# NVlabs/latentfusion

Measured on AMD Instinct MI355X. Metric: pose-optim iters/sec (reconstruct+render+backward), 16 views, 128^3 voxels, higher is better.
Workload: dtype f32

## Files before the change

include/lf_hip.h:

```cpp
#ifndef LF_HIP_H
#define LF_HIP_H

#include <stddef.h>
#include <stdint.h>

#ifdef __cplusplus
extern "C" {
#endif

#define LF_ABI_VERSION 1

#define LF_EINVAL   (-1)
#define LF_EALIGN   (-2)
#define LF_ENOSPC   (-3)

#define LF_EPI_LRELU     1u
#define LF_EPI_PIXELNORM 2u
#define LF_EPI_ADD       4u
#define LF_EPI_DOT       8u

#define LF_MAP_O2C 0
#define LF_MAP_C2O 1
#define LF_MAP_COEFS 20

int lf_abi_version(void);

int lf_device_name(char* buf, int buflen);

int lf_resample3d_fwd(const float* vol, int vol_n, const float* coef, int kind,
                      float* out, int N, int D, int H, int W, int C, void* stream);

size_t lf_resample3d_bwd_coef_scratch_bytes(int N, int D, int H, int W);
int lf_resample3d_bwd_coef(const float* gout, const float* vol, int vol_n, const float* coef,
                           float* gcoef, void* scratch, size_t scratch_bytes,
                           int N, int D, int H, int W, int C, void* stream);
size_t lf_resample3d_bwd_coef_part_scratch_bytes(int N, int part_n, int D, int H, int W);
int lf_resample3d_bwd_coef_part(const float* gout, const float* vol, int vol_n, const float* coef,
                                float* gcoef, void* scratch, size_t scratch_bytes,
                                int N, int D, int H, int W, int C, int part_n, void* stream);

int lf_resample3d_fwd_indexed(const float* vol, int vol_n, const int32_t* vol_idx, const float* coef, int kind,
                              float* out, int N, int D, int H, int W, int C, void* stream);
size_t lf_resample3d_bwd_coef_indexed_scratch_bytes(int N, int part_n, int D, int H, int W);
int lf_resample3d_bwd_coef_indexed(const float* gout, const float* vol, int vol_n, const int32_t* vol_idx, const float* coef,
                                   float* gcoef, void* scratch, size_t scratch_bytes,
                                   int N, int D, int H, int W, int C, int part_n, void* stream);


size_t lf_resample3d_bwd_vol_det_scratch_bytes(int vol_n, int D, int H, int W, int C);
int lf_resample3d_bwd_vol_det(const float* gout, const float* coef, int kind, float* gvol, int vol_n, void* scratch,
                              size_t scratch_bytes, int N, int D, int H, int W, int C, void* stream);

int lf_conv3x3_cout_padded(int Cout);
int lf_conv1x1_cout_padded(int Cout);

int lf_conv3x3_fwd(const float* x, const float* wpack, const float* bias, float* y, float* norm_out,
                   int dims, int N, int D, int H, int W, int Cin, int Cout,
                   float he, unsigned flags, float slope, float eps, void* stream);

int lf_conv1x1_fwd(const float* x, const float* wpack, const float* bias, float* y, float* norm_out,
                   int N, int P, int Cin, int ksl, long x_batch_stride, long x_slice_stride,
                   int Cout, long y_batch_stride, int y_row_stride, int y_slice_channels,
                   long y_slice_stride,
                   float he, unsigned flags, float slope, float eps, void* stream);
int lf_conv1x1_fwd_scaled(const float* x, const float* xscale, const float* wpack, const float* bias, float* y, float* norm_out,
                          int N, int P, int Cin, int ksl, long x_batch_stride, long x_slice_stride,
                          int Cout, long y_batch_stride, int y_row_stride, int y_slice_channels,
                          long y_slice_stride,
                          float he, unsigned flags, float slope, float eps, void* stream);

int lf_conv3x3_bwd_data(const float* gy, const float* wpack_t, float* gx, int dims, int N, int D, int H, int W,
                        int Cin, int Cout, float he, const float* prev_y, const float* prev_norm,
                        unsigned prev_flags, float slope, void* stream);
int lf_conv1x1_bwd_data(const float* gy, const float* wpack_t, float* gx, int N, int P, int Cin, int Cout,
                        long y_batch_stride, int y_row_stride, int y_slice_channels, long y_slice_stride,
                        float he, const float* prev_y, const float* prev_norm, unsigned prev_flags,
                        float slope, float* amax_out, void* stream);

#define LF_AMAX_FLOATS 2048
size_t lf_conv3d_c16_split_wpack_halfs(void);
void lf_conv3d_c16_split_pairs(int* taps28);
int lf_conv3d_c16_split(const float* x, const void* wsplit, const float* bias, float* y, float* norm_out,
                        int N, int D, int H, int W, float he, unsigned flags, float slope, float eps,
                        const float* prev_y, const float* prev_norm, unsigned prev_flags,
                        const float* amax_in, float* amax_out, void* stream);

size_t lf_conv3d_c16_wino_upack_floats(void);
int lf_conv3d_c16_wino(const float* x, const float* upack, const float* bias, float* y, float* norm_out,
                       int N, int D, int H, int W, float he, unsigned flags, float slope, float eps,
                       const float* prev_y, const float* prev_norm, unsigned prev_flags,
                       float* amax_out, void* stream);

size_t lf_conv3d_c16_wino_proj_pack_floats(int D);
int lf_conv3d_c16_wino_projfwd(const float* x, const float* upack, const float* bias, float* y, float* norm_out,
                               int N, int D, int H, int W, float he, unsigned flags, float slope, float eps,
                               const float* proj_wA, const float* proj_bias, float* zp, float* pnorm,
                               float proj_he, unsigned proj_flags, void* stream);

int lf_round_bf16(const float* x, float* y, long n, void* stream);
size_t lf_conv3d_c16_ring_bf16_wpack_elems(void);
int lf_conv3d_c16_ring_bf16(const float* x, const void* wpack, const float* bias, float* y, float* norm_out,
                            int N, int D, int H, int W, float he, unsigned flags, float slope, float eps,
                            const float* addend, int round_out, void* stream);
#define LF_IO_IN_BF16 1
#define LF_IO_OUT_BF16 2
#define LF_IO_ADDEND_BF16 4
int lf_conv3d_c16_ring_bf16_io(const void* x, const void* wpack, const float* bias, void* y, float* norm_out,
                               int N, int D, int H, int W, float he, unsigned flags, float slope, float eps,
                               const void* addend, int round_out, int io, void* stream);

#define LF_RING_ADD_BF16 1u
#define LF_RING_OUT_BF16 2u
#define LF_RING_ROUND 4u
#define LF_RING_EX_NONE 0
#define LF_RING_EX_RH 1
#define LF_RING_EX_BLEND 2
#define LF_RING_EX_ABWD 3
#define LF_RING_EX_BLOCK 4
#define LF_RING_EX_PREV 5
int lf_conv3d_c16_ring_multi(const void* x, int x_bf16, const void* wpack, int ngroups,
                             void* y0, const void* add0, unsigned flags0, void* y1, const void* add1, unsigned flags1,
                             int extra, const void* e0, const void* e1, void* o2,
                             int N, int D, int H, int W, float he, int addend_per_sample, void* stream);
int lf_conv3d_c16_ring_blend(const void* rh, const void* wpack, void* cand, const void* addend, const float* h, const void* upre,
                             float* h_new, void* h_new_bf16, int N, int D, int H, int W, float he, void* stream);

long lf_wino3d_tiles(int N, int D, int H, int W);
int lf_wino3d_input_transform(const float* x, float* V, int N, int D, int H, int W, int C, void* stream);

#define LF_OUT_DEPTH_INNER 0x100u
int lf_wino_fused_cout_padded(int Cout);
size_t lf_wino_fused_scratch_bytes(int dims, int N, int D, int H, int W, int Cout);
int lf_wino_fused_gemm(const float* V, const float* U2, const float* bias, float* y, void* scratch, size_t scratch_bytes,
                       int dims, int N, int D, int H, int W, int Cin, int Cout, float he, unsigned flags, float slope,
                       void* stream);

int lf_wino_f16x3_cin_padded(int Cin);
int lf_wino3d_input_transform_f16x3(const float* x, const float* amax_in, void* V, int N, int D, int H, int W, int C, void* stream);
size_t lf_wino_fused_f16x3_scratch_bytes(int N, int D, int H, int W, int Cout);
int lf_wino_fused_f16x3_gemm(const void* V, const void* U2, int eU, const float* amax_in, const float* bias, float* y,
                             float* amax_out, void* scratch, size_t scratch_bytes, int N, int D, int H, int W, int Cin, int Cout,
                             float he, unsigned flags, float slope, void* stream);

long lf_wino2d_tiles(int N, int H, int W);
int lf_wino2d_input_transform(const float* x, float* V, int N, int H, int W, int C, void* stream);

int lf_wino2d_input_transform_f16x3(const float* x, void* V, int* eV, int N, int H, int W, int C, void* stream);
size_t lf_wino_fused2d_f16x3_scratch_bytes(int N, int H, int W, int Cout);
int lf_wino_fused2d_f16x3_gemm(const void* V, const int* eV, const void* U2, int eU, const float* bias, float* y, void* scratch,
                               size_t scratch_bytes, int N, int H, int W, int Cin, int Cout, float he, unsigned flags, float slope,
                               void* stream);

int lf_gru_stage_a(const float* upre, const float* rpre, int pre_stride, const float* h, float* u, float* rec,
                   long nvox, int Ch, int rec_stride, int rec_off, void* stream);
int lf_gru_stage_b(const float* h, const float* u, const float* cand, float* h_out, float* rec, long nvox, int Ch,
                   int rec_stride, int rec_off, void* stream);
int lf_gru_stage_b_bwd(const float* g, const float* h, const float* u, const float* cand, float* gh, float* gu, float* gc,
                       long n, void* stream);
int lf_gru_stage_a_bwd(const float* gu, const float* grh, const float* u, const float* rpre, const float* h, float* gupre,
                       float* grpre, float* gh, long n, void* stream);
int lf_gru_train_stage_a(const void* rpre, const float* h, void* rh, long n, int bf16, void* stream);
int lf_gru_train_stage_b(const float* h, const void* upre, const void* cand, float* h_out, long n, int bf16, void* stream);
int lf_gru_train_stage_b_bwd(const float* g, const float* h, const void* upre, const void* cand, float* gh1, void* gupre,
                             void* gc, float* acc_u, float* acc_o, long n, int bf16, void* stream);
int lf_gru_train_stage_a_bwd(const void* grh, const void* rpre, const float* h, const float* gh1, void* grpre, float* gh12,
                             float* acc_r, long n, int bf16, void* stream);
int lf_sum_views_bf16(const void* src, float* dst, long n, int views, int accumulate, void* stream);

int lf_resample3d_fwd_io(const void* vol, int vol_n, const float* coef, int kind, void* out, int N, int D, int H, int W,
                         int io, void* stream);
size_t lf_resample3d_bwd_vol_det_io_scratch_bytes(int vol_n, int N, int D, int H, int W);
int lf_resample3d_bwd_vol_det_io(const void* gout, const float* coef, int kind, void* gvol, int vol_n, void* scratch,
                                 size_t scratch_bytes, int N, int D, int H, int W, int io, void* stream);

int lf_occ_input_fwd(const float* z, const float* w, const float* b, float* ta, float* t16, int N, int D, long P, float slope,
                     void* stream);
int lf_occ_input_bwd(const float* gta, const float* ta, const float* gp16, const float* w, const float* g_zs, const float* wocc,
                     float* gz, long rows, float slope, const float* prev_y, const float* prev_norm, unsigned prev_flags,
                     void* stream);
int lf_occ_input_bwd_proj(const float* gta, const float* gp16, const float* w, const float* gp2d, const float* wpack_t, float he_p,
                          const float* wocc, float* gz, int N, int D, long P, float slope,
                          const float* prev_y, const float* prev_norm, unsigned prev_flags, void* stream);
int lf_occ_weight_grad(const float* z, const float* gp2d, const float* wpack_t, float he_p, float* gw, int N, int D, long P, void* stream);
int lf_occ_weight_grad_softmax_bwd(const float* z, const float* gp2d, const float* wpack_t, float he_p, const float* weights,
                                   float* glogits, int N, int D, long P, void* stream);
int lf_occ_head_bwd(const float* gl, const float* w16, float he, const float* y, const float* norm, unsigned flags, float slope,
                    float* g, long rows, void* stream);
int lf_occ_conv17_fwd(const float* t16, const float* w27, float* pre, int N, int D, int H, int W, void* stream);
int lf_occ_conv17_bwd(const float* g, const float* t16, const float* w27, float* gp16, int N, int D, int H, int W, float slope,
                      void* stream);
int lf_column_reduce_sum_fwd(const float* x, float* y, int N, int D, long P, int C, void* stream);
int lf_column_reduce_sum_bwd(const float* gy, float* gx, int N, int D, long P, int C, void* stream);
int lf_column_softmax_fwd(const float* logits, float* weights, float* zdepth, int N, int D, long P, void* stream);
int lf_column_softmax_head_fwd(const float* y, const float* w16, const float* bias, float he, float* weights, float* zdepth,
                               int N, int D, long P, void* stream);
int lf_column_softmax_bwd(const float* weights, const float* gweights, const float* gzdepth, float* glogits,
                          int N, int D, long P, void* stream);
int lf_column_scale_fwd(const float* z, const float* w, float* out, long rows, int C, void* stream);
int lf_column_scale_bwd(const float* gout, const float* z, const float* w, float* gz, float* gw, long rows, int C,
                        void* stream);

#define LF_FUSE_MEAN   0
#define LF_FUSE_MAX    1
#define LF_FUSE_ABSMAX 2
#define LF_FUSE_MEDIAN 3
int lf_fuse_views_fwd(const float* z, float* out, int* idx, int kind, int V, long n, long view_stride, void* stream);
int lf_fuse_views_bwd(const float* g, const int* idx, float* gz, int kind, int V, long n, long view_stride, void* stream);
int lf_fuse_blend_fwd(const float* z, const float* logits, float* weights, float* out, int V, long rows, int C,
                      long z_view_stride, long logit_view_stride, void* stream);
int lf_fuse_blend_bwd(const float* g, const float* z, const float* weights, float* gz, float* glogits, int V, long rows,
                      int C, long z_view_stride, long logit_view_stride, void* stream);

int lf_lstm_cell_fwd(const float* cc, const float* c_cur, float* h_next, float* c_next, long nvox, int Ch, void* stream);
int lf_lstm_cell_bwd(const float* cc, const float* c_cur, const float* gh, const float* gcn, float* gcc, float* gc,
                     long nvox, int Ch, void* stream);

int lf_grid_sample2d_fwd(const float* img, const float* grid, float* out, int N, int C, int H, int W, int Ho, int Wo,
                         int bilinear, int border, void* stream);
int lf_grid_sample2d_bwd(const float* img, const float* grid, const float* gout, float* gimg, float* ggrid,
                         int N, int C, int H, int W, int Ho, int Wo, int bilinear, int border, void* stream);

size_t lf_conv_bwd_weight_scratch_bytes(int dims, int N, int D, int H, int W, int Cin, int Cout);
int lf_conv_bwd_weight(const float* x, const float* gpre, float* gw, void* scratch, size_t scratch_bytes,
                       int dims, int N, int D, int H, int W, int Cin, int Cout, float scale, void* stream);
int lf_conv_bwd_weight_bf16(const float* x, const float* gpre, float* gw, void* scratch, size_t scratch_bytes,
                            int dims, int N, int D, int H, int W, int Cin, int Cout, float scale, void* stream);
int lf_conv_bwd_weight_bf16_io(const void* x, const void* gpre, float* gw, void* scratch, size_t scratch_bytes,
                               int dims, int N, int D, int H, int W, int Cin, int Cout, float scale, int io, void* stream);
size_t lf_conv_bwd_weight_wide_scratch_bytes(int dims, int N, int D, int H, int W, int Cin, int Cout);
int lf_conv_bwd_weight_wide(const float* x, const float* gpre, float* gw, void* scratch, size_t scratch_bytes,
                            int dims, int N, int D, int H, int W, int Cin, int Cout, float scale, void* stream);

size_t lf_epilogue_bwd_c16_scratch_bytes(long rows);
int lf_epilogue_bwd_c16(const void* gy, const void* y, const float* norm, void* gp, float* gbias, void* scratch,
                        size_t scratch_bytes, long rows, unsigned flags, float slope, int io, void* stream);

int lf_lift16_fwd(const float* x, const void* wtab, const float* btab, void* vol, float* norm, long R, long P, int S,
                  float he, float slope, float eps, void* stream);
size_t lf_lift16_bwd_scratch_bytes(int S);
int lf_lift16_bwd(const void* gvol, const void* yvol, const float* norm, const float* x, const void* wtab_t, float* gx, float* gw,
                  float* gb, void* scratch, size_t scratch_bytes, long R, long P, int S, float he, float slope, int round_gx,
                  void* stream);

int lf_proj16_fwd(const void* vol, const void* wtab, const float* bias, float* y, float* norm, long R, long P, int S, float he,
                  float slope, float eps, void* stream);
size_t lf_proj16_bwd_scratch_bytes(int S);
int lf_proj16_bwd(const float* gp, const void* vol, const void* wtab_t, void* gxvol, float* gw, void* scratch, size_t scratch_bytes,
                  long R, long P, int S, float he, void* stream);

int lf_pw16_fwd(const void* x, int x_bf16, const void* w_bf16, const float* bias, float he, unsigned flags, float slope, void* y,
                long rows, void* stream);
size_t lf_pw16_bwd_scratch_bytes(long rows);
int lf_pw16_bwd(const void* gy_bf16, const void* wt_bf16, float he, void* gx, int gx_bf16, float* gbias, void* scratch,
                size_t scratch_bytes, long rows, void* stream);

int lf_pixelnorm_fwd(const float* x, float* y, float* norm_out, long rows, int C, float eps, void* stream);

int lf_epilogue_bwd(const float* gy, const float* y, const float* norm, float* gp,
                    long rows, int C, unsigned flags, float slope, void* stream);
int lf_epilogue_bwd_amax(const float* gy, const float* y, const float* norm, float* gp,
                         long rows, int C, unsigned flags, float slope, float* amax_out, void* stream);

int lf_resize_fwd(const float* x, float* y, int dims, int N, int D, int H, int W, int C, int linear, int up,
                  void* stream);
int lf_resize_bwd(const float* gy, float* gx, int dims, int N, int D, int H, int W, int C, int linear, int up,
                  void* stream);

#define LF_CAM_PARAMS 10
#define LF_CAM_COEFS  24
int lf_camera_coefs(const float* params, const float* intrinsics, float cube_size, float z_span,
                    int crop_h, int crop_w, float* coefs, float* jac, int N, void* stream);
int lf_camera_coefs_bwd(const float* gcoefs, const float* jac, float* gparams, int N, void* stream);

size_t lf_pose_loss_scratch_bytes(int N, int h, int w, int H, int W);
int lf_pose_loss_fwd(const float* logits, const float* coefs, const float* target_depth,
                     const float* target_mask, const float* weights, float* sums, float* losses,
                     float* gsums, void* scratch, size_t scratch_bytes,
                     int N, int h, int w, int H, int W, void* stream);
int lf_pose_loss_bwd(const float* logits, const float* coefs, const float* target_depth,
                     const float* target_mask, const float* gsums, float* glogits, float* gcoefs,
                     void* scratch, size_t scratch_bytes, int N, int h, int w, int H, int W, void* stream);
int lf_pose_loss_fwd_masked(const float* logits, const float* coefs, const float* target_depth,
                            const float* target_mask, const float* weights, float* sums, float* losses,
                            void* scratch, size_t scratch_bytes, int N, int h, int w, int H, int W, void* stream);
int lf_pose_loss_fwd_depth(const float* depth_and_logits, const float* coefs, const float* target_depth,
                           const float* target_mask, const float* weights, float* sums, float* losses,
                           float* gsums, void* scratch, size_t scratch_bytes,
                           int N, int h, int w, int H, int W, void* stream);
int lf_pose_loss_bwd_depth(const float* depth_and_logits, const float* coefs, const float* target_depth,
                           const float* target_mask, const float* gsums, float* gcrop, float* gcoefs,
                           void* scratch, size_t scratch_bytes, int N, int h, int w, int H, int W, void* stream);
int lf_pose_loss_fwd_mt(const float* logits, const float* coefs, const float* target_depth,
                        const float* target_mask, const float* weights, float* sums, float* losses,
                        float* gsums, void* scratch, size_t scratch_bytes,
                        int N, int T, int n, int h, int w, int H, int W, void* stream);
int lf_pose_loss_fwd_masked_mt(const float* logits, const float* coefs, const float* target_depth,
                               const float* target_mask, const float* weights, float* sums, float* losses,
                               void* scratch, size_t scratch_bytes, int N, int T, int n, int h, int w, int H, int W,
                               void* stream);
int lf_pose_loss_bwd_mt(const float* logits, const float* coefs, const float* target_depth,
                        const float* target_mask, const float* gsums, float* glogits, float* gcoefs,
                        void* scratch, size_t scratch_bytes, int N, int T, int n, int h, int w, int H, int W,
                        void* stream);

int lf_adam_step(float* params, const float* grads, float* exp_avg, float* exp_avg_sq,
                 const float* step_size, const float* lr, float bias_correction2_sqrt,
                 float beta1, float beta2, float eps, float weight_decay, int N, int P, void* stream);

int lf_nchw_to_nhwc(const float* src, float* dst, int N, int C, long P, void* stream);
int lf_nhwc_to_nchw(const float* src, float* dst, int N, int C, long P, void* stream);
int lf_lift_unfold(const float* src, const float* norm_or_null, float* dst,
                   int N, long P, int C0, int S, void* stream);
int lf_lift_permute(const float* src, float* dst, int N, long P, int C0, int S, int fold, void* stream);
int lf_lift_norm_unfold(const float* src, void* dst, float* norm_out, int N, long P, int C0, int S, float eps, int out_bf16,
                        void* stream);
int lf_lift_bwd(const void* gvol, const void* yvol, const float* norm, float* gp, int N, long P, int C0, int S, float slope,
                int round_bf16, int io, void* stream);

#ifdef __cplusplus
}
#endif
#endif
```

latentfusion_amd/_lib.py:

```python
import ctypes
import os
from ctypes import c_char_p, c_float, c_int, c_long, c_size_t, c_uint, c_void_p

_HERE = os.path.dirname(os.path.abspath(__file__))
LIB_PATH = os.path.join(_HERE, 'csrc', 'liblf_hip.so')

LF_EPI_LRELU = 1
LF_EPI_PIXELNORM = 2
LF_EPI_ADD = 4
LF_EPI_DOT = 8
LF_RING_ADD_BF16, LF_RING_OUT_BF16, LF_RING_ROUND = 1, 2, 4
LF_RING_EX_NONE, LF_RING_EX_RH, LF_RING_EX_BLEND, LF_RING_EX_ABWD, LF_RING_EX_BLOCK, LF_RING_EX_PREV = 0, 1, 2, 3, 4, 5
LF_OUT_DEPTH_INNER = 0x100
LF_IO_IN_BF16, LF_IO_OUT_BF16, LF_IO_ADDEND_BF16 = 1, 2, 4
LF_MAP_O2C = 0
LF_MAP_C2O = 1
LF_MAP_COEFS = 20
LF_FUSE_MEAN, LF_FUSE_MAX, LF_FUSE_ABSMAX, LF_FUSE_MEDIAN = 0, 1, 2, 3
LF_AMAX_FLOATS = 2048

P = c_void_p
SIGNATURES = {
    'lf_abi_version': (c_int, []),
    'lf_device_name': (c_int, [c_char_p, c_int]),
    'lf_resample3d_fwd': (c_int, [P, c_int, P, c_int, P, c_int, c_int, c_int, c_int, c_int, P]),
    'lf_resample3d_bwd_coef_scratch_bytes': (c_size_t, [c_int, c_int, c_int, c_int]),
    'lf_resample3d_bwd_coef': (c_int, [P, P, c_int, P, P, P, c_size_t, c_int, c_int, c_int, c_int, c_int, P]),
    'lf_resample3d_bwd_coef_part_scratch_bytes': (c_size_t, [c_int, c_int, c_int, c_int, c_int]),
    'lf_resample3d_bwd_coef_part': (c_int, [P, P, c_int, P, P, P, c_size_t, c_int, c_int, c_int, c_int, c_int, c_int, P]),
    'lf_resample3d_fwd_indexed': (c_int, [P, c_int, P, P, c_int, P, c_int, c_int, c_int, c_int, c_int, P]),
    'lf_resample3d_bwd_coef_indexed_scratch_bytes': (c_size_t, [c_int, c_int, c_int, c_int, c_int]),
    'lf_resample3d_bwd_coef_indexed': (c_int, [P, P, c_int, P, P, P, P, c_size_t, c_int, c_int, c_int, c_int, c_int, c_int, P]),
    'lf_resample3d_bwd_vol_det_scratch_bytes': (c_size_t, [c_int, c_int, c_int, c_int, c_int]),
    'lf_resample3d_bwd_vol_det': (c_int, [P, P, c_int, P, c_int, P, c_size_t, c_int, c_int, c_int, c_int, c_int, P]),
    'lf_conv3x3_cout_padded': (c_int, [c_int]),
    'lf_conv1x1_cout_padded': (c_int, [c_int]),
    'lf_conv3x3_fwd': (c_int, [P, P, P, P, P, c_int, c_int, c_int, c_int, c_int, c_int, c_int,
                               c_float, c_uint, c_float, c_float, P]),
    'lf_conv1x1_fwd': (c_int, [P, P, P, P, P, c_int, c_int, c_int, c_int, c_long, c_long, c_int, c_long, c_int,
                               c_int, c_long, c_float, c_uint, c_float, c_float, P]),
    'lf_conv1x1_fwd_scaled': (c_int, [P, P, P, P, P, P, c_int, c_int, c_int, c_int, c_long, c_long, c_int, c_long, c_int,
                                      c_int, c_long, c_float, c_uint, c_float, c_float, P]),
    'lf_conv3x3_bwd_data': (c_int, [P, P, P, c_int, c_int, c_int, c_int, c_int, c_int, c_int, c_float, P, P, c_uint,
                                    c_float, P]),
    'lf_conv1x1_bwd_data': (c_int, [P, P, P, c_int, c_int, c_int, c_int, c_long, c_int, c_int, c_long, c_float, P, P,
                                    c_uint, c_float, P, P]),
    'lf_conv3d_c16_split_wpack_halfs': (c_size_t, []),
    'lf_conv3d_c16_split_pairs': (None, [P]),
    'lf_conv3d_c16_split': (c_int, [P, P, P, P, P, c_int, c_int, c_int, c_int, c_float, c_uint, c_float, c_float, P, P,
                                    c_uint, P, P, P]),
    'lf_conv3d_c16_wino_upack_floats': (c_size_t, []),
    'lf_conv3d_c16_wino': (c_int, [P, P, P, P, P, c_int, c_int, c_int, c_int, c_float, c_uint, c_float, c_float, P, P,
                                   c_uint, P, P]),
    'lf_conv3d_c16_wino_proj_pack_floats': (c_size_t, [c_int]),
    'lf_conv3d_c16_wino_projfwd': (c_int, [P, P, P, P, P, c_int, c_int, c_int, c_int, c_float, c_uint, c_float, c_float,
                                           P, P, P, P, c_float, c_uint, P]),
    'lf_round_bf16': (c_int, [P, P, c_long, P]),
    'lf_conv3d_c16_ring_bf16_wpack_elems': (c_size_t, []),
    'lf_conv3d_c16_ring_bf16': (c_int, [P, P, P, P, P, c_int, c_int, c_int, c_int, c_float, c_uint, c_float, c_float, P, c_int, P]),
    'lf_conv3d_c16_ring_bf16_io': (c_int, [P, P, P, P, P, c_int, c_int, c_int, c_int, c_float, c_uint, c_float, c_float, P, c_int, c_int, P]),
    'lf_conv3d_c16_ring_multi': (c_int, [P, c_int, P, c_int, P, P, c_uint, P, P, c_uint, c_int, P, P, P, c_int, c_int, c_int, c_int, c_float, c_int, P]),
    'lf_conv3d_c16_ring_blend': (c_int, [P, P, P, P, P, P, P, P, c_int, c_int, c_int, c_int, c_float, P]),
    'lf_wino3d_tiles': (c_long, [c_int, c_int, c_int, c_int]),
    'lf_wino3d_input_transform': (c_int, [P, P, c_int, c_int, c_int, c_int, c_int, P]),
    'lf_wino_fused_cout_padded': (c_int, [c_int]),
    'lf_wino_fused_scratch_bytes': (c_size_t, [c_int, c_int, c_int, c_int, c_int, c_int]),
    'lf_wino_fused_gemm': (c_int, [P, P, P, P, P, c_size_t, c_int, c_int, c_int, c_int, c_int, c_int, c_int, c_float, c_uint, c_float, P]),
    'lf_wino_f16x3_cin_padded': (c_int, [c_int]),
    'lf_wino3d_input_transform_f16x3': (c_int, [P, P, P, c_int, c_int, c_int, c_int, c_int, P]),
    'lf_wino_fused_f16x3_scratch_bytes': (c_size_t, [c_int, c_int, c_int, c_int, c_int]),
    'lf_wino_fused_f16x3_gemm': (c_int, [P, P, c_int, P, P, P, P, P, c_size_t, c_int, c_int, c_int, c_int, c_int, c_int,
                                         c_float, c_uint, c_float, P]),
    'lf_wino2d_tiles': (c_long, [c_int, c_int, c_int]),
    'lf_wino2d_input_transform': (c_int, [P, P, c_int, c_int, c_int, c_int, P]),
    'lf_wino2d_input_transform_f16x3': (c_int, [P, P, P, c_int, c_int, c_int, c_int, P]),
    'lf_wino_fused2d_f16x3_scratch_bytes': (c_size_t, [c_int, c_int, c_int, c_int]),
    'lf_wino_fused2d_f16x3_gemm': (c_int, [P, P, P, c_int, P, P, P, c_size_t, c_int, c_int, c_int, c_int, c_int, c_float, c_uint,
                                           c_float, P]),
    'lf_gru_stage_a': (c_int, [P, P, c_int, P, P, P, c_long, c_int, c_int, c_int, P]),
    'lf_gru_stage_b': (c_int, [P, P, P, P, P, c_long, c_int, c_int, c_int, P]),
    'lf_lstm_cell_fwd': (c_int, [P, P, P, P, c_long, c_int, P]),
    'lf_lstm_cell_bwd': (c_int, [P, P, P, P, P, P, c_long, c_int, P]),
    'lf_gru_stage_b_bwd': (c_int, [P, P, P, P, P, P, P, c_long, P]),
    'lf_gru_stage_a_bwd': (c_int, [P, P, P, P, P, P, P, P, c_long, P]),
    'lf_gru_train_stage_a': (c_int, [P, P, P, c_long, c_int, P]),
    'lf_gru_train_stage_b': (c_int, [P, P, P, P, c_long, c_int, P]),
    'lf_gru_train_stage_b_bwd': (c_int, [P, P, P, P, P, P, P, P, P, c_long, c_int, P]),
    'lf_gru_train_stage_a_bwd': (c_int, [P, P, P, P, P, P, P, c_long, c_int, P]),
    'lf_lift16_fwd': (c_int, [P, P, P, P, P, c_long, c_long, c_int, c_float, c_float, c_float, P]),
    'lf_lift16_bwd_scratch_bytes': (c_size_t, [c_int]),
    'lf_lift16_bwd': (c_int, [P, P, P, P, P, P, P, P, P, c_size_t, c_long, c_long, c_int, c_float, c_float, c_int, P]),
    'lf_proj16_fwd': (c_int, [P, P, P, P, P, c_long, c_long, c_int, c_float, c_float, c_float, P]),
    'lf_proj16_bwd_scratch_bytes': (c_size_t, [c_int]),
    'lf_proj16_bwd': (c_int, [P, P, P, P, P, P, c_size_t, c_long, c_long, c_int, c_float, P]),
    'lf_sum_views_bf16': (c_int, [P, P, c_long, c_int, c_int, P]),
    'lf_occ_input_fwd': (c_int, [P, P, P, P, P, c_int, c_int, c_long, c_float, P]),
    'lf_occ_input_bwd': (c_int, [P, P, P, P, P, P, P, c_long, c_float, P, P, c_uint, P]),
    'lf_occ_conv17_fwd': (c_int, [P, P, P, c_int, c_int, c_int, c_int, P]),
    'lf_occ_conv17_bwd': (c_int, [P, P, P, P, c_int, c_int, c_int, c_int, c_float, P]),
    'lf_column_reduce_sum_fwd': (c_int, [P, P, c_int, c_int, c_long, c_int, P]),
    'lf_column_reduce_sum_bwd': (c_int, [P, P, c_int, c_int, c_long, c_int, P]),
    'lf_column_softmax_fwd': (c_int, [P, P, P, c_int, c_int, c_long, P]),
    'lf_occ_input_bwd_proj': (c_int, [P, P, P, P, P, c_float, P, P, c_int, c_int, c_long, c_float, P, P, c_uint, P]),
    'lf_occ_weight_grad': (c_int, [P, P, P, c_float, P, c_int, c_int, c_long, P]),
    'lf_pw16_fwd': (c_int, [P, c_int, P, P, c_float, c_uint, c_float, P, c_long, P]),
    'lf_pw16_bwd_scratch_bytes': (c_size_t, [c_long]),
    'lf_pw16_bwd': (c_int, [P, P, c_float, P, c_int, P, P, c_size_t, c_long, P]),
    'lf_occ_weight_grad_softmax_bwd': (c_int, [P, P, P, c_float, P, P, c_int, c_int, c_long, P]),
    'lf_occ_head_bwd': (c_int, [P, P, c_float, P, P, c_uint, c_float, P, c_long, P]),
    'lf_column_softmax_head_fwd': (c_int, [P, P, P, c_float, P, P, c_int, c_int, c_long, P]),
    'lf_column_softmax_bwd': (c_int, [P, P, P, P, c_int, c_int, c_long, P]),
    'lf_column_scale_fwd': (c_int, [P, P, P, c_long, c_int, P]),
    'lf_column_scale_bwd': (c_int, [P, P, P, P, P, c_long, c_int, P]),
    'lf_fuse_views_fwd': (c_int, [P, P, P, c_int, c_int, c_long, c_long, P]),
    'lf_fuse_views_bwd': (c_int, [P, P, P, c_int, c_int, c_long, c_long, P]),
    'lf_fuse_blend_fwd': (c_int, [P, P, P, P, c_int, c_long, c_int, c_long, c_long, P]),
    'lf_fuse_blend_bwd': (c_int, [P, P, P, P, P, c_int, c_long, c_int, c_long, c_long, P]),
    'lf_grid_sample2d_fwd': (c_int, [P, P, P, c_int, c_int, c_int, c_int, c_int, c_int, c_int, c_int, P]),
    'lf_grid_sample2d_bwd': (c_int, [P, P, P, P, P, c_int, c_int, c_int, c_int, c_int, c_int, c_int, c_int, P]),
    'lf_conv_bwd_weight_scratch_bytes': (c_size_t, [c_int, c_int, c_int, c_int, c_int, c_int, c_int]),
    'lf_conv_bwd_weight': (c_int, [P, P, P, P, c_size_t, c_int, c_int, c_int, c_int, c_int, c_int, c_int, c_float, P]),
    'lf_conv_bwd_weight_bf16': (c_int, [P, P, P, P, c_size_t, c_int, c_int, c_int, c_int, c_int, c_int, c_int, c_float, P]),
    'lf_conv_bwd_weight_bf16_io': (c_int, [P, P, P, P, c_size_t, c_int, c_int, c_int, c_int, c_int, c_int, c_int, c_float, c_int, P]),
    'lf_conv_bwd_weight_wide_scratch_bytes': (c_size_t, [c_int, c_int, c_int, c_int, c_int, c_int, c_int]),
    'lf_conv_bwd_weight_wide': (c_int, [P, P, P, P, c_size_t, c_int, c_int, c_int, c_int, c_int, c_int, c_int, c_float, P]),
    'lf_pixelnorm_fwd': (c_int, [P, P, P, c_long, c_int, c_float, P]),
    'lf_epilogue_bwd': (c_int, [P, P, P, P, c_long, c_int, c_uint, c_float, P]),
    'lf_epilogue_bwd_amax': (c_int, [P, P, P, P, c_long, c_int, c_uint, c_float, P, P]),
    'lf_epilogue_bwd_c16_scratch_bytes': (c_size_t, [c_long]),
    'lf_epilogue_bwd_c16': (c_int, [P, P, P, P, P, P, c_size_t, c_long, c_uint, c_float, c_int, P]),
    'lf_resample3d_fwd_io': (c_int, [P, c_int, P, c_int, P, c_int, c_int, c_int, c_int, c_int, P]),
    'lf_resample3d_bwd_vol_det_io_scratch_bytes': (c_size_t, [c_int, c_int, c_int, c_int, c_int]),
    'lf_resample3d_bwd_vol_det_io': (c_int, [P, P, c_int, P, c_int, P, c_size_t, c_int, c_int, c_int, c_int, c_int, P]),
    'lf_resize_fwd': (c_int, [P, P, c_int, c_int, c_int, c_int, c_int, c_int, c_int, c_int, P]),
    'lf_resize_bwd': (c_int, [P, P, c_int, c_int, c_int, c_int, c_int, c_int, c_int, c_int, P]),
    'lf_camera_coefs': (c_int, [P, P, c_float, c_float, c_int, c_int, P, P, c_int, P]),
    'lf_camera_coefs_bwd': (c_int, [P, P, P, c_int, P]),
    'lf_pose_loss_scratch_bytes': (c_size_t, [c_int, c_int, c_int, c_int, c_int]),
    'lf_pose_loss_fwd': (c_int, [P, P, P, P, P, P, P, P, P, c_size_t, c_int, c_int, c_int, c_int, c_int, P]),
    'lf_pose_loss_bwd': (c_int, [P, P, P, P, P, P, P, P, c_size_t, c_int, c_int, c_int, c_int, c_int, P]),
    'lf_pose_loss_fwd_depth': (c_int, [P, P, P, P, P, P, P, P, P, c_size_t, c_int, c_int, c_int, c_int, c_int, P]),
    'lf_pose_loss_bwd_depth': (c_int, [P, P, P, P, P, P, P, P, c_size_t, c_int, c_int, c_int, c_int, c_int, P]),
    'lf_pose_loss_fwd_masked': (c_int, [P, P, P, P, P, P, P, P, c_size_t, c_int, c_int, c_int, c_int, c_int, P]),
    'lf_pose_loss_fwd_mt': (c_int, [P, P, P, P, P, P, P, P, P, c_size_t, c_int, c_int, c_int, c_int, c_int, c_int, c_int, P]),
    'lf_pose_loss_fwd_masked_mt': (c_int, [P, P, P, P, P, P, P, P, c_size_t, c_int, c_int, c_int, c_int, c_int, c_int, c_int,
                                           P]),
    'lf_pose_loss_bwd_mt': (c_int, [P, P, P, P, P, P, P, P, c_size_t, c_int, c_int, c_int, c_int, c_int, c_int, c_int, P]),
    'lf_adam_step': (c_int, [P, P, P, P, P, P, c_float, c_float, c_float, c_float, c_float, c_int, c_int, P]),
    'lf_nchw_to_nhwc': (c_int, [P, P, c_int, c_int, c_long, P]),
    'lf_nhwc_to_nchw': (c_int, [P, P, c_int, c_int, c_long, P]),
    'lf_lift_unfold': (c_int, [P, P, P, c_int, c_long, c_int, c_int, P]),
    'lf_lift_permute': (c_int, [P, P, c_int, c_long, c_int, c_int, c_int, P]),
    'lf_lift_norm_unfold': (c_int, [P, P, P, c_int, c_long, c_int, c_int, c_float, c_int, P]),
    'lf_lift_bwd': (c_int, [P, P, P, P, c_int, c_long, c_int, c_int, c_float, c_int, c_int, P]),
}

EXPERIMENTAL_SIGNATURES = {
    'lf_set_tuning': (c_int, [c_int, c_int]),
    'lf_resample3d_bwd_vol': (c_int, [P, P, c_int, P, c_int, c_int, c_int, c_int, c_int, c_int, P]),
    'lf_conv3d_c16_wino_projbwd': (c_int, [P, P, c_float, P, P, c_uint, P, P, c_int, c_int, c_int, c_int, c_float, c_float,
                                           P, P, c_uint, P]),
    'lf_conv3d_c16_wino_split_upack_halfs': (c_size_t, []),
    'lf_conv3d_c16_wino_split': (c_int, [P, P, P, P, P, c_int, c_int, c_int, c_int, c_float, c_uint, c_float, c_float, P, P,
                                         c_uint, P, P, P]),
    'lf_conv3d_c16_bf16_wpack_elems': (c_size_t, []),
    'lf_conv3d_c16_bf16': (c_int, [P, P, P, P, P, c_int, c_int, c_int, c_int, c_float, c_uint, c_float, c_float, c_int, P]),
    'lf_wino3d_output_transform': (c_int, [P, P, P, P, c_int, c_int, c_int, c_int, c_int, c_float, c_uint, c_float, c_float, P]),
    'lf_wino2d_output_transform': (c_int, [P, P, P, P, c_int, c_int, c_int, c_int, c_float, c_uint, c_float, c_float, P]),
}

_lib = None


class LFHipError(RuntimeError):
    pass


def lib():
    global _lib
    if _lib is not None:
        return _lib
    if not os.path.exists(LIB_PATH):
        try:
            from .csrc import build as _build
            _build.build(verbose=False)
        except Exception as e:
            raise LFHipError(f'liblf_hip.so is missing at {LIB_PATH} and could not be built: {e}') from e
    import torch
    try:
        handle = ctypes.CDLL(LIB_PATH)
    except OSError as e:
        raise LFHipError(f'cannot load {LIB_PATH}: {e}') from e
    for name, (res, args) in list(SIGNATURES.items()) + list(EXPERIMENTAL_SIGNATURES.items()):
        try:
            fn = getattr(handle, name)
        except AttributeError as e:
            raise LFHipError(f'{LIB_PATH} does not export {name}') from e
        fn.restype = res
        fn.argtypes = args
    if handle.lf_abi_version() != 1:
        raise LFHipError('liblf_hip.so ABI version mismatch')
    _lib = handle
    return _lib


_ERR = {-1: 'LF_EINVAL (bad size/flag combination)', -2: 'LF_EALIGN (alignment / channel count)',
        -3: 'LF_ENOSPC (scratch too small)'}


BYTE_LOG = None
_PENDING = [0]


def note_bytes(t, scratch=False):
    if BYTE_LOG is not None and not scratch:
        n = t.numel() * t.element_size()
        try:
            n = min(n, t.untyped_storage().nbytes() - t.storage_offset() * t.element_size())
        except Exception:
            pass
        _PENDING[0] += n


def check(rc, what):
    if BYTE_LOG is not None:
        e = BYTE_LOG.setdefault(what, [0, 0])
        e[0] += 1
        e[1] += _PENDING[0]
        _PENDING[0] = 0
    if rc != 0:
        raise LFHipError(f'{what} failed: {_ERR.get(rc, "hipError " + str(rc))}')
```

latentfusion_amd/csrc/build.py:

```python
import os
import subprocess
import sys

HERE = os.path.dirname(os.path.abspath(__file__))
SOURCES = ['resample.hip', 'conv.hip', 'pointwise.hip', 'image.hip', 'optim.hip', 'resize.hip', 'conv_split.hip', 'conv_wino.hip', 'wgrad.hip', 'sample2d.hip', 'gru.hip', 'wino_gemm.hip', 'reduce.hip', 'wino_fused.hip', 'conv_bf16.hip', 'occlusion.hip', 'conv_gru.hip', 'lift_mfma.hip', 'pw16.hip', 'wino_fused_f16x3.hip', 'wgrad_wide.hip']
LIB = os.path.join(HERE, 'liblf_hip.so')
EXTRA = {'conv_split.hip': ['-fno-slp-vectorize'], 'conv_gru.hip': ['-fno-slp-vectorize']}
FLAGS = ['--offload-arch=gfx950', '-O3', '-std=c++17', '-fPIC', '-fno-gpu-rdc', '-Wall', '-Wno-unused-function']


def _hipcc():
    for cand in (os.environ.get('HIPCC'), '/opt/rocm/bin/hipcc', 'hipcc'):
        if cand and (os.path.isabs(cand) and os.path.exists(cand) or not os.path.isabs(cand)):
            return cand
    raise RuntimeError('hipcc not found')


def needs_build():
    if not os.path.exists(LIB):
        return True
    t = os.path.getmtime(LIB)
    deps = [os.path.join(HERE, s) for s in SOURCES if os.path.exists(os.path.join(HERE, s))]
    deps += [os.path.join(HERE, f) for f in os.listdir(HERE) if f.endswith(('.h', '.inc'))]
    deps += [os.path.join(HERE, '..', '..', 'include', 'lf_hip.h'), os.path.join(HERE, '..', '..', 'include', 'lf_hip_experimental.h')]
    return any(os.path.getmtime(d) > t for d in deps)


def build(force=False, verbose=True):
    if not force and not needs_build():
        return LIB
    hipcc = _hipcc()
    objs = []
    procs = []
    for src in SOURCES:
        path = os.path.join(HERE, src)
        if not os.path.exists(path):
            continue
        obj = os.path.join(HERE, src.replace('.hip', '.o'))
        objs.append(obj)
        cmd = [hipcc, '-x', 'hip', '-c', path, '-o', obj] + FLAGS + EXTRA.get(src, [])
        procs.append((cmd, subprocess.Popen(cmd, stdout=subprocess.PIPE, stderr=subprocess.STDOUT)))
    for cmd, p in procs:
        out, _ = p.communicate()
        if p.returncode != 0:
            raise RuntimeError('hipcc failed: ' + ' '.join(cmd) + '\n' + out.decode())
        if verbose and out.strip():
            print(out.decode())
    cmd = [hipcc, '-shared', '-fPIC', '--offload-arch=gfx950', '-o', LIB] + objs
    r = subprocess.run(cmd, stdout=subprocess.PIPE, stderr=subprocess.STDOUT)
    if r.returncode != 0:
        raise RuntimeError('link failed:\n' + r.stdout.decode())
    if verbose:
        print('built', LIB)
    return LIB


if __name__ == '__main__':
    build(force='--force' in sys.argv)
```

latentfusion_amd/csrc/lf_common.h:

```cpp
#pragma once
#include <hip/hip_runtime.h>
#include <stdint.h>
#include "../../include/lf_hip.h"
#include "../../include/lf_hip_experimental.h"

#define LF_WAVE 64

typedef float f32x4 __attribute__((ext_vector_type(4)));

static inline void lf_clear_error() { (void)hipGetLastError(); }

static inline int lf_launch_status() {
  hipError_t e = hipGetLastError();
  return (int)e;
}

static inline bool lf_aligned16(const void* p) { return (((uintptr_t)p) & 15u) == 0; }

#include <atomic>
typedef std::atomic<unsigned long long> lf_devmask_t;
static inline hipError_t lf_ensure_dyn_lds(lf_devmask_t& done, const void* fn, int bytes) {
  int dev = 0;
  if (hipGetDevice(&dev) != hipSuccess) dev = 0;
  const unsigned long long bit = 1ull << (dev & 63);
  if (done.load(std::memory_order_acquire) & bit) return hipSuccess;
  const hipError_t e = hipFuncSetAttribute(fn, hipFuncAttributeMaxDynamicSharedMemorySize, bytes);
  if (e == hipSuccess) done.fetch_or(bit, std::memory_order_release);
  return e;
}

__device__ __forceinline__ float lf_wave_sum(float v) {
#pragma unroll
  for (int o = 32; o > 0; o >>= 1) v += __shfl_xor(v, o, 64);
  return v;
}

#define LF_AMAX_SLOTS 64
#define LF_AMAX_STRIDE 32
static_assert(LF_AMAX_FLOATS == LF_AMAX_SLOTS * LF_AMAX_STRIDE, "lf_hip.h: LF_AMAX_FLOATS");

__device__ __forceinline__ void lf_amax_publish(float* base, float wave_max, int lane) {
  if (lane == 0 && wave_max > 0.f)
    atomicMax((unsigned int*)(base + (blockIdx.x % LF_AMAX_SLOTS) * LF_AMAX_STRIDE), __float_as_uint(wave_max));
}

__device__ __forceinline__ float lf_amax_read(const float* base, int lane) {
  float m = base[(lane % LF_AMAX_SLOTS) * LF_AMAX_STRIDE];
#pragma unroll
  for (int o = 32; o > 0; o >>= 1) m = fmaxf(m, __shfl_xor(m, o, 64));
  return m;
}

__device__ __forceinline__ float lf_lrelu(float v, float slope) { return v > 0.f ? v : v * slope; }

int lf_internal_ring_bf16_set_wgs(int v);
int lf_internal_fused_set_cfg(int v);
```

latentfusion_amd/csrc/resample.hip:

```cpp
#include "lf_common.h"
#include <type_traits>

namespace {

typedef unsigned u32x4_t __attribute__((ext_vector_type(4)));

struct Tap {
  int x0, y0, z0, x1, y1, z1;
  float tx, ty, tz;
  float mx, my, mz;
};

__device__ __forceinline__ float lattice01(int i, int size, float step) {
  return (i < size / 2) ? step * (float)i : 1.f - step * (float)(size - 1 - i);
}

struct Steps { float w, h, d; };

template <int KIND>
__device__ __forceinline__ void eval_grid(const float* __restrict__ cf, int x, int y, int z,
                                          int W, int H, int D, Steps st, float& gx, float& gy, float& gz,
                                          float& a, float& b, float& k) {
  a = lattice01(x, W, st.w);
  b = lattice01(y, H, st.h);
  k = lattice01(z, D, st.d);
  if (KIND == LF_MAP_O2C) {
    const float ak = a * k, bk = b * k;
    gx = cf[0] + cf[3] * a + cf[6] * b + cf[9] * k + cf[12] * ak + cf[15] * bk;
    gy = cf[1] + cf[4] * a + cf[7] * b + cf[10] * k + cf[13] * ak + cf[16] * bk;
    gz = cf[2] + cf[5] * a + cf[8] * b + cf[11] * k + cf[14] * ak + cf[17] * bk;
  } else {
    const float lx = 2.f * a - 1.f, ly = 2.f * b - 1.f, lz = 2.f * k - 1.f;
    const float n0 = cf[0] * lx + cf[1] * ly + cf[2] * lz + cf[3];
    const float n1 = cf[4] * lx + cf[5] * ly + cf[6] * lz + cf[7];
    const float n2 = cf[8] * lx + cf[9] * ly + cf[10] * lz + cf[11];
    const float dn = cf[12] * lx + cf[13] * ly + cf[14] * lz + cf[15];
    gx = n0 / dn;
    gy = n1 / dn;
    gz = n2;
  }
}

__device__ __forceinline__ void unnormalize_clip(float g, int size, float& pos, float& mult) {
  float p = ((g + 1.f) * (float)size - 1.f) * 0.5f;
  const float hi = (float)(size - 1);
  mult = (p > 0.f && p < hi) ? 0.5f * (float)size : 0.f;
  p = fminf(fmaxf(p, 0.f), hi);
  pos = p;
}

__device__ __forceinline__ Tap make_tap(float gx, float gy, float gz, int W, int H, int D) {
  Tap t;
  float px, py, pz;
  unnormalize_clip(gx, W, px, t.mx);
  unnormalize_clip(gy, H, py, t.my);
  unnormalize_clip(gz, D, pz, t.mz);
  if (!(px == px)) px = 0.f;
  if (!(py == py)) py = 0.f;
  if (!(pz == pz)) pz = 0.f;
  const float fx = floorf(px), fy = floorf(py), fz = floorf(pz);
  t.tx = px - fx; t.ty = py - fy; t.tz = pz - fz;
  t.x0 = (int)fx; t.y0 = (int)fy; t.z0 = (int)fz;
  t.x1 = min(t.x0 + 1, W - 1); t.y1 = min(t.y0 + 1, H - 1); t.z1 = min(t.z0 + 1, D - 1);
  return t;
}

__device__ __forceinline__ unsigned xcd_contiguous(unsigned b, unsigned nb) {
  return (nb % 8 == 0) ? (b % 8) * (nb / 8) + b / 8 : b;
}

static int bwd_vox_per_block(long nvox, int N) {
  long v = nvox * N / 2048;
  int p = 64;
  while (p < 4096 && p * 2 <= v) p <<= 1;
  return p;
}
struct BwdTile { int lx, ly, lz, ntx, nty, ntz; };
static BwdTile bwd_tile(int vpb, int D, int H, int W) {
  int lg = 0;
  while ((1 << lg) < vpb) ++lg;
  BwdTile t;
  t.lx = (lg + 2) / 3; t.ly = (lg + 1) / 3; t.lz = lg / 3;
  t.ntx = (W + (1 << t.lx) - 1) >> t.lx; t.nty = (H + (1 << t.ly) - 1) >> t.ly; t.ntz = (D + (1 << t.lz) - 1) >> t.lz;
  return t;
}

__global__ void __launch_bounds__(256) resample_bwd_coef_reduce(const float* __restrict__ partial,
                                                                int nblk, float* __restrict__ gcoef) {
  const int n = blockIdx.x;
  __shared__ double red[256];
  const int comp = threadIdx.x % 18;
  const int grp = threadIdx.x / 18;
  double s = 0.0;
  if (grp < 14)
    for (int b = grp; b < nblk; b += 14) s += (double)partial[((long)n * nblk + b) * 18 + comp];
  red[threadIdx.x] = (grp < 14) ? s : 0.0;
  __syncthreads();
  if (threadIdx.x < 18) {
    double tot = 0.0;
    for (int g = 0; g < 14; ++g) tot += red[g * 18 + threadIdx.x];
    gcoef[(long)n * 18 + threadIdx.x] = (float)tot;
  }
}

template <int KIND>
__global__ void __launch_bounds__(256) resample_bwd_vol_kernel(
    const float* __restrict__ gout, const float* __restrict__ coef, float* __restrict__ gvol,
    long gvol_bstride, int N, int D, int H, int W, int C, Steps st) {
  const long per_sample = (long)D * H * W * C;
  const int n = blockIdx.y;
  const float* cf = coef + (long)n * LF_MAP_COEFS;
  for (long idx = (long)blockIdx.x * blockDim.x + threadIdx.x; idx < per_sample;
       idx += (long)gridDim.x * blockDim.x) {
    const int c = (int)(idx % C);
    long v = idx / C;
    const int x = (int)(v % W); v /= W;
    const int y = (int)(v % H);
    const int z = (int)(v / H);
    float gx, gy, gz, a, b, k;
    eval_grid<KIND>(cf, x, y, z, W, H, D, st, gx, gy, gz, a, b, k);
    const Tap t = make_tap(gx, gy, gz, W, H, D);
    const float go = gout[(long)n * per_sample + idx];
    float* base = gvol + (long)n * gvol_bstride + c;
    const long sW = C, sH = (long)W * C, sD = (long)H * W * C;
    const float wx1 = t.tx, wx0 = 1.f - t.tx, wy1 = t.ty, wy0 = 1.f - t.ty, wz1 = t.tz, wz0 = 1.f - t.tz;
    atomicAdd(base + t.z0 * sD + t.y0 * sH + t.x0 * sW, go * (wx0 * wy0 * wz0));
    atomicAdd(base + t.z0 * sD + t.y0 * sH + t.x1 * sW, go * (wx1 * wy0 * wz0));
    atomicAdd(base + t.z0 * sD + t.y1 * sH + t.x0 * sW, go * (wx0 * wy1 * wz0));
    atomicAdd(base + t.z0 * sD + t.y1 * sH + t.x1 * sW, go * (wx1 * wy1 * wz0));
    atomicAdd(base + t.z1 * sD + t.y0 * sH + t.x0 * sW, go * (wx0 * wy0 * wz1));
    atomicAdd(base + t.z1 * sD + t.y0 * sH + t.x1 * sW, go * (wx1 * wy0 * wz1));
    atomicAdd(base + t.z1 * sD + t.y1 * sH + t.x0 * sW, go * (wx0 * wy1 * wz1));
    atomicAdd(base + t.z1 * sD + t.y1 * sH + t.x1 * sW, go * (wx1 * wy1 * wz1));
  }
}

typedef unsigned u32;

struct Tap32 {
  u32 o000, o001, o010, o011, o100, o101, o110, o111;
  float tx, ty, tz, mx, my, mz;
};

__device__ __forceinline__ void axis_tap(float g, int size, u32 stride, u32& o0, u32& d1, float& t, float& m) {
  float p;
  unnormalize_clip(g, size, p, m);
  if (!(p == p)) p = 0.f;
  const float f = floorf(p);
  t = p - f;
  const int i0 = (int)f;
  o0 = (u32)i0 * stride;
  d1 = (i0 + 1 <= size - 1) ? stride : 0u;
}

__device__ __forceinline__ Tap32 make_tap32(float gx, float gy, float gz, int W, int H, int D, u32 rec_bytes) {
  Tap32 t;
  u32 x0, dx, y0, dy, z0, dz;
  axis_tap(gx, W, rec_bytes, x0, dx, t.tx, t.mx);
  axis_tap(gy, H, rec_bytes * (u32)W, y0, dy, t.ty, t.my);
  axis_tap(gz, D, rec_bytes * (u32)W * (u32)H, z0, dz, t.tz, t.mz);
  const u32 b00 = z0 + y0, b01 = b00 + dy, b10 = b00 + dz, b11 = b01 + dz;
  t.o000 = b00 + x0; t.o001 = t.o000 + dx;
  t.o010 = b01 + x0; t.o011 = t.o010 + dx;
  t.o100 = b10 + x0; t.o101 = t.o100 + dx;
  t.o110 = b11 + x0; t.o111 = t.o110 + dx;
  return t;
}

__device__ __forceinline__ f32x4 ldrec(__amdgpu_buffer_rsrc_t rs, u32 off) {
  return __builtin_bit_cast(f32x4, __builtin_amdgcn_raw_buffer_load_b128(rs, (int)off, 0, 0));
}

typedef __bf16 bf16x4r __attribute__((ext_vector_type(4)));
typedef unsigned u32x2_t __attribute__((ext_vector_type(2)));
template <bool B16>
__device__ __forceinline__ f32x4 ldrec_t(__amdgpu_buffer_rsrc_t rs, u32 off) {
  if constexpr (B16)
    return __builtin_convertvector(__builtin_bit_cast(bf16x4r, __builtin_amdgcn_raw_buffer_load_b64(rs, (int)off, 0, 0)), f32x4);
  else
    return __builtin_bit_cast(f32x4, __builtin_amdgcn_raw_buffer_load_b128(rs, (int)off, 0, 0));
}

__device__ __forceinline__ float quad_sum4(float v) {
  const float a = v + __int_as_float(__builtin_amdgcn_update_dpp(0, __float_as_int(v), 0xB1, 0xF, 0xF, true));
  return a + __int_as_float(__builtin_amdgcn_update_dpp(0, __float_as_int(a), 0x4E, 0xF, 0xF, true));
}

__device__ __forceinline__ long vol_offset(int n, long vol_bstride, const int* __restrict__ vol_idx, int vol_n) {
  const int v = vol_idx[n];
  return (long)(v < 0 ? 0 : (v >= vol_n ? vol_n - 1 : v)) * vol_bstride;
}

#define GATHER_KERNEL(stem) stem##_kernel
#define GATHER_TABLE_PARAMS
#define GATHER_VOL_OFFSET ((long)n * vol_bstride)
#include "resample_gather.inc"
#undef GATHER_KERNEL
#undef GATHER_TABLE_PARAMS
#undef GATHER_VOL_OFFSET
#define GATHER_KERNEL(stem) stem##_indexed_kernel
#define GATHER_TABLE_PARAMS const int* __restrict__ vol_idx, int vol_n,
#define GATHER_VOL_OFFSET vol_offset(n, vol_bstride, vol_idx, vol_n)
#include "resample_gather.inc"
#undef GATHER_KERNEL
#undef GATHER_TABLE_PARAMS
#undef GATHER_VOL_OFFSET

template <int KIND>
__global__ void __launch_bounds__(256) resample_fwd_c16_dedup_kernel(
    const float* __restrict__ vol, long vol_bstride, const float* __restrict__ coef,
    float* __restrict__ out, int D, int H, int W, int nbx, int nby, int nbz, Steps st) {
  __shared__ u32x4_t tapo[4][64];
  __shared__ f32x4 tapf[4][64];
  const int lane = threadIdx.x & 63, wave = threadIdx.x >> 6;
  const int n = blockIdx.z / nbz, bz = blockIdx.z - n * nbz;
  const int x0 = ((blockIdx.x << 2) + wave) << 2, y0 = blockIdx.y << 2, z0 = bz << 2;
  const u32 sample_bytes = (u32)D * (u32)H * (u32)W * 64u;
  const __amdgpu_buffer_rsrc_t rs = __builtin_amdgcn_make_buffer_rsrc((void*)(vol + (long)n * vol_bstride), 0, sample_bytes, 0x00020000);
  const __amdgpu_buffer_rsrc_t ro = __builtin_amdgcn_make_buffer_rsrc((void*)(out + (long)n * D * H * W * 16), 0, sample_bytes, 0x00020000);
  const float* cf = coef + n * LF_MAP_COEFS;
  {
    const int x = x0 + (lane & 3), y = y0 + ((lane >> 2) & 3), z = z0 + (lane >> 4);
    const bool live = x < W && y < H && z < D;
    float gx, gy, gz, a, b, k;
    eval_grid<KIND>(cf, live ? x : 0, live ? y : 0, live ? z : 0, W, H, D, st, gx, gy, gz, a, b, k);
    const Tap32 t = make_tap32(gx, gy, gz, W, H, D, 64u);
    u32x4_t o;
    o[0] = live ? t.o000 : 0xffffffffu;
    o[1] = t.o001 - t.o000; o[2] = t.o010 - t.o000; o[3] = t.o100 - t.o000;
    tapo[wave][lane] = o;
    tapf[wave][lane] = (f32x4){t.tx, t.ty, t.tz, 0.f};
  }
  asm volatile("s_waitcnt lgkmcnt(0)" ::: "memory");
  const int q = lane & 3, vq = lane >> 2;
  const u32 co = (u32)q * 16u;
#pragma unroll
  for (int i = 0; i < 4; ++i) {
    const int vi = 16 * i + vq;
    const u32x4_t o = tapo[wave][vi];
    const f32x4 f = tapf[wave][vi];
    if (o[0] == 0xffffffffu) continue;
    const u32 b00 = o[0] + co, b01 = b00 + o[2], b10 = b00 + o[3], b11 = b01 + o[3];
    const f32x4 v000 = ldrec(rs, b00), v001 = ldrec(rs, b00 + o[1]), v010 = ldrec(rs, b01), v011 = ldrec(rs, b01 + o[1]);
    const f32x4 v100 = ldrec(rs, b10), v101 = ldrec(rs, b10 + o[1]), v110 = ldrec(rs, b11), v111 = ldrec(rs, b11 + o[1]);
    const float wx1 = f[0], wx0 = 1.f - f[0], wy1 = f[1], wy0 = 1.f - f[1], wz1 = f[2], wz0 = 1.f - f[2];
    const float w000 = wx0 * wy0 * wz0, w001 = wx1 * wy0 * wz0, w010 = wx0 * wy1 * wz0, w011 = wx1 * wy1 * wz0;
    const float w100 = wx0 * wy0 * wz1, w101 = wx1 * wy0 * wz1, w110 = wx0 * wy1 * wz1, w111 = wx1 * wy1 * wz1;
    f32x4 r;
#pragma unroll
    for (int e = 0; e < 4; ++e) {
      float acc = v000[e] * w000;
      asm("v_fmac_f32 %0, %1, %2" : "+v"(acc) : "v"(v001[e]), "v"(w001));
      asm("v_fmac_f32 %0, %1, %2" : "+v"(acc) : "v"(v010[e]), "v"(w010));
      asm("v_fmac_f32 %0, %1, %2" : "+v"(acc) : "v"(v011[e]), "v"(w011));
      asm("v_fmac_f32 %0, %1, %2" : "+v"(acc) : "v"(v100[e]), "v"(w100));
// ... 562 lines not shown
  for (int j = 0; j < 16; ++j) {
    const int r = wv * 64 + j * 4 + grp;
    const int lx = r % STX, ly = (r / STX) % STY, lz = r / (STX * STY);
    const int x = tx0 + lx, y = ty0 + ly, z = tz0 + lz;
    if (x < W && y < H && z < D) {
      char* dst = (char*)gvol + (n_out * nvox + (((long)z * H + y) * W + x)) * OREC;
      const float o = (float)((double)(long long)acc[r * 16 + ch] * inv);
      if constexpr (OUT16) ((__bf16*)dst)[ch] = __builtin_convertvector((f32x4){o, o, o, o}, bf16x4r)[0];
      else ((float*)dst)[ch] = o;
    }
  }
}

int g_splat_chunk_cap = 0;
inline int splat_bin_chunk(int N, long nvox) {
  long cv = (512L << 20) / (nvox * 32);
  if (cv < 1) cv = 1;
  if (g_splat_chunk_cap > 0 && cv > g_splat_chunk_cap) cv = g_splat_chunk_cap;
  return (int)(cv < N ? cv : N);
}

int g_splat_variant = 2;

bool pow2(int v) { return v > 0 && (v & (v - 1)) == 0; }

Steps make_steps(int D, int H, int W) {
  Steps st;
  st.w = W > 1 ? 1.0f / (float)(W - 1) : 0.f;
  st.h = H > 1 ? 1.0f / (float)(H - 1) : 0.f;
  st.d = D > 1 ? 1.0f / (float)(D - 1) : 0.f;
  return st;
}

}

struct FwdPlan {
  bool vec;
  int lpt, tlx, tly, tlz, nbz;
  dim3 grid;
  Steps st;
};
static int fwd_plan(const float* vol, const float* out, int N, int D, int H, int W, int C, FwdPlan& p) {
  if ((long)D * H * W >= 0x7fffffffL) return LF_EINVAL;
  p.vec = (C % 4 == 0) && lf_aligned16(vol) && lf_aligned16(out);
  const int lpv = p.vec ? C / 4 : C;
  p.lpt = lpv < 256 ? lpv : 256;
  int lg = 0;
  while ((2 << lg) * p.lpt <= 256) ++lg;
  if (lg >= 6) { p.tlx = (lg + 2) / 3; p.tly = (lg + 1) / 3; p.tlz = lg / 3; }
  else         { p.tlx = lg < 2 ? lg : 2; p.tly = lg - p.tlx < 2 ? lg - p.tlx : 2; p.tlz = lg - p.tlx - p.tly; }
  p.nbz = (D + (1 << p.tlz) - 1) >> p.tlz;
  const int nby = (H + (1 << p.tly) - 1) >> p.tly;
  if ((long)p.nbz * N > 65535 || nby > 65535) return LF_EINVAL;
  p.grid = dim3((unsigned)((W + (1 << p.tlx) - 1) >> p.tlx), (unsigned)nby, (unsigned)(p.nbz * N));
  p.st = make_steps(D, H, W);
  return 0;
}

#define LAUNCH_BY_KIND(KERNEL, GRID, ...)                                                                   \
  do {                                                                                                      \
    if (kind == LF_MAP_O2C) hipLaunchKernelGGL((KERNEL<LF_MAP_O2C>), GRID, dim3(256), 0, s, __VA_ARGS__);   \
    else                    hipLaunchKernelGGL((KERNEL<LF_MAP_C2O>), GRID, dim3(256), 0, s, __VA_ARGS__);   \
  } while (0)
extern "C" int lf_resample3d_fwd(const float* vol, int vol_n, const float* coef, int kind, float* out,
                                 int N, int D, int H, int W, int C, void* stream) {
  lf_clear_error();
  if (N <= 0 || D <= 0 || H <= 0 || W <= 0 || C <= 0) return LF_EINVAL;
  if (vol_n != 1 && vol_n != N) return LF_EINVAL;
  if (kind != LF_MAP_O2C && kind != LF_MAP_C2O) return LF_EINVAL;
  const long bstride = vol_n == 1 ? 0 : (long)D * H * W * C;
  FwdPlan p;
  if (int e = fwd_plan(vol, out, N, D, H, W, C, p)) return e;
  hipStream_t s = (hipStream_t)stream;
  if (g_resample_variant == 4 && p.vec && C == 16 && (long)D * H * W * 64 < 0xffffffffL && W <= 65535) {
    const int ntx = (W + LT_X - 1) / LT_X, nty = (H + LT_Y - 1) / LT_Y, ntz = (D + LT_Z - 1) / LT_Z;
    const long nwg = (long)ntx * nty * ntz * N;
    if (nwg > 0x7fffffffL) return LF_EINVAL;
    LAUNCH_BY_KIND(resample_fwd_staged_kernel, dim3((unsigned)nwg), vol, bstride, coef, out, D, H, W, ntx, nty, ntz, p.st);
    return lf_launch_status();
  }
  if (g_resample_variant == 5 && p.vec && C == 16 && (long)D * H * W * 64 < 0xffffffffL) {
    const int nbz4 = (D + 3) >> 2, nbx16 = (W + 15) >> 4, nby4 = (H + 3) >> 2;
    if ((long)nbz4 * N > 65535 || nby4 > 65535) return LF_EINVAL;
    dim3 g5((unsigned)nbx16, (unsigned)nby4, (unsigned)(nbz4 * N));
    LAUNCH_BY_KIND(resample_fwd_c16_dedup_kernel, g5, vol, bstride, coef, out, D, H, W, nbx16, nby4, nbz4, p.st);
    return lf_launch_status();
  }
  if (g_resample_variant >= 3 && p.vec && C == 16 && (long)D * H * W * 64 < 0xffffffffL) {
    LAUNCH_BY_KIND(resample_fwd_c16_kernel, p.grid, vol, bstride, coef, out, D, H, W, p.nbz, p.st);
  } else if (g_resample_variant >= 2 && p.vec && (long)D * H * W * C * 4 < 0xffffffffL) {
    LAUNCH_BY_KIND(resample_fwd_lean_kernel, p.grid, vol, bstride, coef, out, D, H, W, C, p.lpt, p.tlx, p.tly, p.tlz, p.nbz, p.st);
  } else {
#define LAUNCH(K, V) hipLaunchKernelGGL((resample_fwd_kernel<K, V>), p.grid, dim3(256), 0, s, vol, bstride, coef, out, N, D, H, W, C, p.lpt, p.tlx, p.tly, p.tlz, p.nbz, p.st)
    if (kind == LF_MAP_O2C) { if (p.vec) LAUNCH(LF_MAP_O2C, 4); else LAUNCH(LF_MAP_O2C, 1); }
    else                    { if (p.vec) LAUNCH(LF_MAP_C2O, 4); else LAUNCH(LF_MAP_C2O, 1); }
#undef LAUNCH
  }
  return lf_launch_status();
}

static long staged_bwd_blocks(int D, int H, int W) {
  const long nt = (long)((W + LT_X - 1) / LT_X) * ((H + LT_Y - 1) / LT_Y) * ((D + LT_Z - 1) / LT_Z);
  return (nt + STAGED_TPW - 1) / STAGED_TPW;
}

static size_t bwd_coef_scratch_bytes(int N, int part_n, int D, int H, int W) {
  const long nvox = (long)D * H * W;
  const int vpb = bwd_vox_per_block(nvox, part_n);
  const BwdTile bt = bwd_tile(vpb, D, H, W);
  const long nblk = (long)bt.ntx * bt.nty * bt.ntz;
  const long nblk_staged = staged_bwd_blocks(D, H, W);
  return (size_t)N * (nblk > nblk_staged ? nblk : nblk_staged) * 18 * sizeof(float);
}

extern "C" size_t lf_resample3d_bwd_coef_scratch_bytes(int N, int D, int H, int W) {
  return bwd_coef_scratch_bytes(N, N, D, H, W);
}

extern "C" size_t lf_resample3d_bwd_coef_part_scratch_bytes(int N, int part_n, int D, int H, int W) {
  if (N <= 0 || part_n <= 0) return 0;
  return bwd_coef_scratch_bytes(N, part_n, D, H, W);
}

struct BwdCoefPlan {
  long nvox;
  int vpb, nblk, lpv;
  BwdTile bt;
  bool vec;
  dim3 grid;
  Steps st;
};
static int bwd_coef_plan(const float* gout, const float* vol, size_t scratch_bytes, int N, int part_n, int D, int H, int W, int C,
                         BwdCoefPlan& p) {
  if (scratch_bytes < bwd_coef_scratch_bytes(N, part_n, D, H, W)) return LF_ENOSPC;
  if ((long)D * H * W >= 0x7fffffffL) return LF_EINVAL;
  p.nvox = (long)D * H * W;
  p.vpb = bwd_vox_per_block(p.nvox, part_n);
  p.bt = bwd_tile(p.vpb, D, H, W);
  const long nblk_l = (long)p.bt.ntx * p.bt.nty * p.bt.ntz;
  if (nblk_l * N > 0x7fffffffL) return LF_EINVAL;
  p.nblk = (int)nblk_l;
  p.grid = dim3((unsigned)(nblk_l * N));
  p.vec = (C % 4 == 0) && lf_aligned16(gout) && lf_aligned16(vol);
  const int groups = p.vec ? C / 4 : C;
  p.lpv = 1;
  while (p.lpv < groups) p.lpv <<= 1;
  if (p.lpv > 64) return LF_EINVAL;
  p.st = make_steps(D, H, W);
  return 0;
}

static int bwd_coef_finish(const float* partial, int nblk, float* gcoef, int N, hipStream_t s) {
  if (int e = lf_launch_status()) return e;
  hipLaunchKernelGGL(resample_bwd_coef_reduce, dim3(N), dim3(256), 0, s, partial, nblk, gcoef);
  return lf_launch_status();
}

static int bwd_coef_launch(const float* gout, const float* vol, int vol_n, const float* coef,
                           float* gcoef, void* scratch, size_t scratch_bytes,
                           int N, int part_n, int D, int H, int W, int C, void* stream) {
  if (N <= 0 || D <= 0 || H <= 0 || W <= 0 || C <= 0) return LF_EINVAL;
  if (vol_n != 1 && vol_n != N) return LF_EINVAL;
  BwdCoefPlan p;
  if (int e = bwd_coef_plan(gout, vol, scratch_bytes, N, part_n, D, H, W, C, p)) return e;
  const long bstride = vol_n == 1 ? 0 : p.nvox * C;
  hipStream_t s = (hipStream_t)stream;
  float* partial = (float*)scratch;
  if (g_resample_variant == 4 && p.vec && C == 16 && p.nvox * 64 < 0xffffffffL && W <= 65535) {
    const int ntx = (W + LT_X - 1) / LT_X, nty = (H + LT_Y - 1) / LT_Y, ntz = (D + LT_Z - 1) / LT_Z;
    const long nb = staged_bwd_blocks(D, H, W);
    if (nb * N > 0x7fffffffL) return LF_EINVAL;
    hipLaunchKernelGGL((resample_bwd_coef_staged_kernel<STAGED_TPW>), dim3((unsigned)(nb * N)), dim3(256), 0, s, gout, vol, bstride, coef,
                       partial, (int)nb, D, H, W, ntx, nty, ntz, p.st);
    return bwd_coef_finish(partial, (int)nb, gcoef, N, s);
  }
  if (g_resample_variant >= 2 && p.vec && C == 16 && p.vpb >= 64 && p.nvox * 64 < 0xffffffffL) {
    const int v = g_bwd_coef_variant;
    const bool big = p.vpb >= 256;
#define LAUNCH(...) hipLaunchKernelGGL((__VA_ARGS__), p.grid, dim3(256), 0, s, gout, vol, bstride, coef, partial, p.nblk, p.vpb, p.bt, D, H, W, p.st)
    if (v == 1)              LAUNCH(resample_bwd_coef_c16_kernel<1, 1>);
    else if (v == 2)         LAUNCH(resample_bwd_coef_c16_kernel<1, 2>);
    else if (v == 3)         LAUNCH(resample_bwd_coef_c16_kernel<4, 2>);
    else if (v == 6 && big)  LAUNCH(resample_bwd_coef_c16_dedup_kernel<2, 1>);
    else if (v == 7 && big)  LAUNCH(resample_bwd_coef_c16_dedup_kernel<1, 1>);
    else if (v == 8 && big)  LAUNCH(resample_bwd_coef_c16_dedup_kernel<2, 4>);
    else if (v == 9 && big)  LAUNCH(resample_bwd_coef_c16_dedup_kernel<1, 5>);
    else if (v == 10 && big) LAUNCH(resample_bwd_coef_c16_dedup_kernel<2, 1, true>);
    else if (v == 11 && big) LAUNCH(resample_bwd_coef_c16_dedup_kernel<1, 1, true>);
    else if (v == 4)         LAUNCH(resample_bwd_coef_c16_kernel<6, 1>);
    else                     LAUNCH(resample_bwd_coef_c16_kernel<8, 1>);
#undef LAUNCH
  } else if (p.vec) {
    hipLaunchKernelGGL((resample_bwd_coef_kernel<4>), p.grid, dim3(256), 0, s, gout, vol, bstride, coef, partial, p.nblk, p.vpb, p.bt, N, D, H, W, C, p.lpv, p.st);
  } else {
    hipLaunchKernelGGL((resample_bwd_coef_kernel<1>), p.grid, dim3(256), 0, s, gout, vol, bstride, coef, partial, p.nblk, p.vpb, p.bt, N, D, H, W, C, p.lpv, p.st);
  }
  return bwd_coef_finish(partial, p.nblk, gcoef, N, s);
}

extern "C" int lf_resample3d_bwd_coef(const float* gout, const float* vol, int vol_n, const float* coef,
                                      float* gcoef, void* scratch, size_t scratch_bytes,
                                      int N, int D, int H, int W, int C, void* stream) {
  lf_clear_error();
  return bwd_coef_launch(gout, vol, vol_n, coef, gcoef, scratch, scratch_bytes, N, N, D, H, W, C, stream);
}

extern "C" int lf_resample3d_bwd_coef_part(const float* gout, const float* vol, int vol_n, const float* coef,
                                           float* gcoef, void* scratch, size_t scratch_bytes,
                                           int N, int D, int H, int W, int C, int part_n, void* stream) {
  lf_clear_error();
  if (!gout || !vol || !coef || !gcoef || !scratch) return LF_EINVAL;
  if (part_n <= 0 || N <= 0) return LF_EINVAL;
  return bwd_coef_launch(gout, vol, vol_n, coef, gcoef, scratch, scratch_bytes, N, part_n, D, H, W, C, stream);
}

extern "C" int lf_resample3d_fwd_indexed(const float* vol, int vol_n, const int* vol_idx, const float* coef, int kind, float* out,
                                         int N, int D, int H, int W, int C, void* stream) {
  lf_clear_error();
  if (!vol || !vol_idx || !coef || !out) return LF_EINVAL;
  if (N <= 0 || D <= 0 || H <= 0 || W <= 0 || C <= 0 || vol_n < 1) return LF_EINVAL;
  if (kind != LF_MAP_O2C && kind != LF_MAP_C2O) return LF_EINVAL;
  if (((uintptr_t)vol_idx & 3) != 0) return LF_EALIGN;
  const long bstride = (long)D * H * W * C;
  FwdPlan p;
  if (int e = fwd_plan(vol, out, N, D, H, W, C, p)) return e;
  hipStream_t s = (hipStream_t)stream;
  if (g_resample_variant >= 3 && p.vec && C == 16 && (long)D * H * W * 64 < 0xffffffffL) {
    LAUNCH_BY_KIND(resample_fwd_c16_indexed_kernel, p.grid, vol, bstride, vol_idx, vol_n, coef, out, D, H, W, p.nbz, p.st);
  } else if (g_resample_variant >= 2 && p.vec && (long)D * H * W * C * 4 < 0xffffffffL) {
    LAUNCH_BY_KIND(resample_fwd_lean_indexed_kernel, p.grid, vol, bstride, vol_idx, vol_n, coef, out, D, H, W, C, p.lpt, p.tlx, p.tly, p.tlz, p.nbz, p.st);
  } else {
#define LAUNCH(K, V) hipLaunchKernelGGL((resample_fwd_indexed_kernel<K, V>), p.grid, dim3(256), 0, s, vol, bstride, vol_idx, vol_n, coef, out, N, D, H, W, C, p.lpt, p.tlx, p.tly, p.tlz, p.nbz, p.st)
    if (kind == LF_MAP_O2C) { if (p.vec) LAUNCH(LF_MAP_O2C, 4); else LAUNCH(LF_MAP_O2C, 1); }
    else                    { if (p.vec) LAUNCH(LF_MAP_C2O, 4); else LAUNCH(LF_MAP_C2O, 1); }
#undef LAUNCH
  }
  return lf_launch_status();
}
#undef LAUNCH_BY_KIND

extern "C" size_t lf_resample3d_bwd_coef_indexed_scratch_bytes(int N, int part_n, int D, int H, int W) {
  if (N <= 0 || part_n <= 0) return 0;
  return bwd_coef_scratch_bytes(N, part_n, D, H, W);
}

extern "C" int lf_resample3d_bwd_coef_indexed(const float* gout, const float* vol, int vol_n, const int* vol_idx, const float* coef,
                                              float* gcoef, void* scratch, size_t scratch_bytes,
                                              int N, int D, int H, int W, int C, int part_n, void* stream) {
  lf_clear_error();
  if (!gout || !vol || !vol_idx || !coef || !gcoef || !scratch) return LF_EINVAL;
  if (part_n <= 0 || N <= 0 || vol_n < 1) return LF_EINVAL;
  if (D <= 0 || H <= 0 || W <= 0 || C <= 0) return LF_EINVAL;
  if (((uintptr_t)vol_idx & 3) != 0) return LF_EALIGN;
  BwdCoefPlan p;
  if (int e = bwd_coef_plan(gout, vol, scratch_bytes, N, part_n, D, H, W, C, p)) return e;
  const long bstride = p.nvox * C;
  hipStream_t s = (hipStream_t)stream;
  float* partial = (float*)scratch;
  if (g_resample_variant >= 2 && p.vec && C == 16 && p.vpb >= 64 && p.nvox * 64 < 0xffffffffL) {
    if (p.vpb >= 256)
      hipLaunchKernelGGL((resample_bwd_coef_c16_dedup_indexed_kernel<2, 1, true>), p.grid, dim3(256), 0, s, gout, vol, bstride, vol_idx, vol_n, coef, partial, p.nblk, p.vpb, p.bt, D, H, W, p.st);
    else
      hipLaunchKernelGGL((resample_bwd_coef_c16_indexed_kernel<8, 1>), p.grid, dim3(256), 0, s, gout, vol, bstride, vol_idx, vol_n, coef, partial, p.nblk, p.vpb, p.bt, D, H, W, p.st);
  } else if (p.vec) {
    hipLaunchKernelGGL((resample_bwd_coef_indexed_kernel<4>), p.grid, dim3(256), 0, s, gout, vol, bstride, vol_idx, vol_n, coef, partial, p.nblk, p.vpb, p.bt, N, D, H, W, C, p.lpv, p.st);
  } else {
    hipLaunchKernelGGL((resample_bwd_coef_indexed_kernel<1>), p.grid, dim3(256), 0, s, gout, vol, bstride, vol_idx, vol_n, coef, partial, p.nblk, p.vpb, p.bt, N, D, H, W, C, p.lpv, p.st);
  }
  return bwd_coef_finish(partial, p.nblk, gcoef, N, s);
}

extern "C" int lf_resample3d_bwd_vol(const float* gout, const float* coef, int kind, float* gvol, int vol_n,
                                     int N, int D, int H, int W, int C, void* stream) {
  lf_clear_error();
  if (N <= 0 || D <= 0 || H <= 0 || W <= 0 || C <= 0) return LF_EINVAL;
  if (vol_n != 1 && vol_n != N) return LF_EINVAL;
  const long bstride = vol_n == 1 ? 0 : (long)D * H * W * C;
  const long items = (long)D * H * W * C;
  dim3 grid((unsigned)min((items + 255) / 256, (long)65535 * 16), N), block(256);
  hipStream_t s = (hipStream_t)stream;
  if (kind == LF_MAP_O2C)
    hipLaunchKernelGGL((resample_bwd_vol_kernel<LF_MAP_O2C>), grid, block, 0, s, gout, coef, gvol, bstride, N, D, H, W, C, make_steps(D, H, W));
  else if (kind == LF_MAP_C2O)
    hipLaunchKernelGGL((resample_bwd_vol_kernel<LF_MAP_C2O>), grid, block, 0, s, gout, coef, gvol, bstride, N, D, H, W, C, make_steps(D, H, W));
  else
    return LF_EINVAL;
  return lf_launch_status();
}

#ifdef STAGE_TS
extern "C" int lf_debug_stage_ts(void* dst) {
  return (int)hipMemcpyFromSymbol(dst, HIP_SYMBOL(g_stage_ts), sizeof(unsigned long long) * 256 * 16, 0, hipMemcpyDeviceToHost);
}
#endif

extern "C" int lf_set_tuning(int key, int value) {
  if (key == 1) {
    const int prev = g_resample_variant;
    if (value >= 1 && value <= 5) g_resample_variant = value;
    return prev;
  }
  if (key == 4) {
    const int prev = g_splat_variant;
    if (value >= 1 && value <= 4) g_splat_variant = value;
    return prev;
  }
  if (key == 6) {
    const int prev = g_splat_chunk_cap;
    if (value >= 0) g_splat_chunk_cap = value;
    return prev;
  }
  if (key == 3) return lf_internal_fused_set_cfg(value);
  if (key == 5) return lf_internal_ring_bf16_set_wgs(value);
  if (key == 2) {
    const int prev = g_bwd_coef_variant;
    if (value >= 1 && value <= 11) g_bwd_coef_variant = value;
    return prev;
  }
  return LF_EINVAL;
}

extern "C" size_t lf_resample3d_bwd_vol_det_scratch_bytes(int vol_n, int D, int H, int W, int C) {
  if (vol_n <= 0 || D <= 0 || H <= 0 || W <= 0 || C <= 0) return 0;
  return (size_t)vol_n * D * H * W * C * sizeof(long long) + 256;
}

extern "C" int lf_resample3d_bwd_vol_det(const float* gout, const float* coef, int kind, float* gvol, int vol_n, void* scratch,
                                         size_t scratch_bytes, int N, int D, int H, int W, int C, void* stream) {
  lf_clear_error();
  if (N <= 0 || D <= 0 || H <= 0 || W <= 0 || C <= 0) return LF_EINVAL;
  if ((vol_n != 1 && vol_n != N) || (kind != LF_MAP_O2C && kind != LF_MAP_C2O)) return LF_EINVAL;
  const long items = (long)D * H * W * C, total = items * vol_n;
  if (scratch == nullptr || scratch_bytes < lf_resample3d_bwd_vol_det_scratch_bytes(vol_n, D, H, W, C)) return LF_ENOSPC;
  if ((((uintptr_t)scratch) & 7u) != 0) return LF_EALIGN;
  hipStream_t s = (hipStream_t)stream;
  const long ng = items * N;
  const int nbx = (W + 3) / 4, nby = (H + 3) / 4, nbz = (D + 3) / 4;
  const long nblk = (long)nbx * nby * nbz;
  const int ntx = (W + STX - 1) / STX, nty = (H + STY - 1) / STY, ntz = (D + STZ - 1) / STZ;
  const int nsx = (nbx + 3) / 4, nsy = (nby + 3) / 4, nsz = (nbz + 3) / 4, nsb = nsx * nsy * nsz;
  if (g_splat_variant >= 2 && C == 16 && lf_aligned16(gout) && lf_aligned16(gvol) && D < 0x7fff && H < 0x7fff && W < 0x7fff &&
      nblk < 0x7fffffffL / 4 && (long)ntx * nty * ntz < 0x7fffffffL && N <= 65535 &&
      scratch_bytes >= 256 + (size_t)N * (nblk + nsb) * sizeof(uint3)) {
    unsigned* amax = (unsigned*)scratch;
    uint3* bbox = (uint3*)((char*)scratch + 256);
    uint3* sbox = bbox + (size_t)N * nblk;
    hipError_t e = hipMemsetAsync(scratch, 0, 256, s);
    if (e != hipSuccess) return (int)e;
    hipLaunchKernelGGL(absmax_kernel, dim3((unsigned)min((ng + 255) / 256, 4096L)), dim3(256), 0, s, gout, ng, amax);
    const Steps stp = make_steps(D, H, W);
    const dim3 gb((unsigned)((nblk + 3) / 4), (unsigned)N), gs2((unsigned)((nsb + 3) / 4), (unsigned)N),
        gt((unsigned)((long)ntx * nty * ntz), (unsigned)vol_n);
    if (kind == LF_MAP_O2C)
      hipLaunchKernelGGL((splat_bbox_kernel<LF_MAP_O2C>), gb, dim3(256), 0, s, coef, bbox, (int)nblk, nbx, nby, D, H, W, stp);
    else
      hipLaunchKernelGGL((splat_bbox_kernel<LF_MAP_C2O>), gb, dim3(256), 0, s, coef, bbox, (int)nblk, nbx, nby, D, H, W, stp);
    hipLaunchKernelGGL(splat_bbox2_kernel, gs2, dim3(256), 0, s, bbox, sbox, (int)nblk, nsb, nbx, nby, nbz, nsx, nsy);
    if (kind == LF_MAP_O2C)
      hipLaunchKernelGGL((splat_tile_kernel<LF_MAP_O2C>), gt, dim3(256), 0, s, gout, coef, bbox, sbox, amax, gvol, vol_n, N, (int)nblk, nsb,
                         nbx, nby, nbz, nsx, nsy, ntx, nty, D, H, W, stp);
    else
      hipLaunchKernelGGL((splat_tile_kernel<LF_MAP_C2O>), gt, dim3(256), 0, s, gout, coef, bbox, sbox, amax, gvol, vol_n, N, (int)nblk, nsb,
                         nbx, nby, nbz, nsx, nsy, ntx, nty, D, H, W, stp);
    return lf_launch_status();
  }
  unsigned long long* acc = (unsigned long long*)scratch;
  unsigned* amax = (unsigned*)((char*)scratch + (size_t)total * sizeof(long long));
  hipError_t e = hipMemsetAsync(scratch, 0, (size_t)total * sizeof(long long) + 256, s);
  if (e != hipSuccess) return (int)e;
  hipLaunchKernelGGL(absmax_kernel, dim3((unsigned)min((ng + 255) / 256, 4096L)), dim3(256), 0, s, gout, ng, amax);
  int st = lf_launch_status();
  if (st) return st;
  const long bstride = vol_n == 1 ? 0 : items;
  dim3 grid((unsigned)min((items + 255) / 256, (long)65535 * 16), N), block(256);
  if (kind == LF_MAP_O2C)
    hipLaunchKernelGGL((resample_bwd_vol_fixed_kernel<LF_MAP_O2C>), grid, block, 0, s, gout, coef, acc, bstride, amax, N, D, H, W, C, make_steps(D, H, W));
  else
    hipLaunchKernelGGL((resample_bwd_vol_fixed_kernel<LF_MAP_C2O>), grid, block, 0, s, gout, coef, acc, bstride, amax, N, D, H, W, C, make_steps(D, H, W));
  st = lf_launch_status();
  if (st) return st;
  hipLaunchKernelGGL(fixed_to_float_kernel, dim3((unsigned)((total + 255) / 256)), dim3(256), 0, s, (const long long*)acc, amax, gvol, total);
  return lf_launch_status();
}

extern "C" int lf_resample3d_fwd_io(const void* vol, int vol_n, const float* coef, int kind, void* out,
                                    int N, int D, int H, int W, int io, void* stream) {
  lf_clear_error();
  if (N <= 0 || D <= 0 || H <= 0 || W <= 0 || io < 0 || io > 3) return LF_EINVAL;
  if ((vol_n != 1 && vol_n != N) || (kind != LF_MAP_O2C && kind != LF_MAP_C2O)) return LF_EINVAL;
  if (!lf_aligned16(vol) || !lf_aligned16(out)) return LF_EALIGN;
  if ((long)D * H * W * 64 >= 0xffffffffL) return LF_EINVAL;
  const long bstride = vol_n == 1 ? 0 : (long)D * H * W * 16;
  const int nbz4 = (D + 3) >> 2;
  if ((long)nbz4 * N > 65535 || ((H + 3) >> 2) > 65535) return LF_EINVAL;
  dim3 g4((unsigned)((W + 3) >> 2), (unsigned)((H + 3) >> 2), (unsigned)(nbz4 * N)), block(256);
  const Steps st = make_steps(D, H, W);
  typedef void (*kern_t)(const float*, long, const float*, float*, int, int, int, int, Steps);
  static const kern_t kerns[2][4] = {
      {resample_fwd_c16_kernel<LF_MAP_O2C, 0>, resample_fwd_c16_kernel<LF_MAP_O2C, 1>, resample_fwd_c16_kernel<LF_MAP_O2C, 2>, resample_fwd_c16_kernel<LF_MAP_O2C, 3>},
      {resample_fwd_c16_kernel<LF_MAP_C2O, 0>, resample_fwd_c16_kernel<LF_MAP_C2O, 1>, resample_fwd_c16_kernel<LF_MAP_C2O, 2>, resample_fwd_c16_kernel<LF_MAP_C2O, 3>}};
  hipLaunchKernelGGL(kerns[kind == LF_MAP_O2C ? 0 : 1][io], g4, block, 0, (hipStream_t)stream, (const float*)vol, bstride, coef, (float*)out, D, H, W, nbz4, st);
  return lf_launch_status();
}

static bool splat_binned_ok(int vol_n, int N, int D, int H, int W) {
  if (g_splat_variant == 3 || W > 1024 || H > 1024 || D > 4096) return false;
  return vol_n == N || splat_bin_chunk(N, (long)D * H * W) == N;
}

extern "C" size_t lf_resample3d_bwd_vol_det_io_scratch_bytes(int vol_n, int N, int D, int H, int W) {
  if (N <= 0 || D <= 0 || H <= 0 || W <= 0) return 0;
  const long nbx = (W + 3) / 4, nby = (H + 3) / 4, nbz = (D + 3) / 4;
  const long nsb = ((nbx + 3) / 4) * ((nby + 3) / 4) * ((nbz + 3) / 4);
  const size_t boxes = 256 + (size_t)N * (size_t)(nbx * nby * nbz + nsb) * sizeof(uint3);
  const long nvox = (long)D * H * W;
  const long nt = (long)((W + STX - 1) / STX) * ((H + STY - 1) / STY) * ((D + STZ - 1) / STZ);
  const long cv = splat_bin_chunk(N, nvox);
  const size_t lists = 256 + (size_t)(3 * cv * nt * 4) + (size_t)(cv * nvox * 32);
  return boxes > lists ? boxes : lists;
}

extern "C" int lf_resample3d_bwd_vol_det_io(const void* gout, const float* coef, int kind, void* gvol, int vol_n, void* scratch,
                                            size_t scratch_bytes, int N, int D, int H, int W, int io, void* stream) {
  lf_clear_error();
  if (N <= 0 || D <= 0 || H <= 0 || W <= 0 || io < 0 || io > 3) return LF_EINVAL;
  if ((vol_n != 1 && vol_n != N) || (kind != LF_MAP_O2C && kind != LF_MAP_C2O)) return LF_EINVAL;
  if (scratch == nullptr || scratch_bytes < lf_resample3d_bwd_vol_det_io_scratch_bytes(vol_n, N, D, H, W)) return LF_ENOSPC;
  if ((((uintptr_t)scratch) & 7u) != 0 || !lf_aligned16(gout) || !lf_aligned16(gvol)) return LF_EALIGN;
  hipStream_t s = (hipStream_t)stream;
  const long ng = (long)D * H * W * 16 * N;
  if (splat_binned_ok(vol_n, N, D, H, W)) {
    const long nvox = (long)D * H * W;
    const int ntx = (W + STX - 1) / STX, nty = (H + STY - 1) / STY, ntz = (D + STZ - 1) / STZ;
    const long nt = (long)ntx * nty * ntz;
    if (nvox >= 0xffffffffL || nt >= 0x7fffffffL || N > 65535) return LF_EINVAL;
    const int cv = splat_bin_chunk(N, nvox);
    const long cap = nvox * 8;
    unsigned* amax = (unsigned*)scratch;
    unsigned* cnt = (unsigned*)((char*)scratch + 256);
    unsigned* cur = cnt + (size_t)cv * nt;
    unsigned* off = cur + (size_t)cv * nt;
    unsigned* list = off + (size_t)cv * nt;
    hipError_t e = hipMemsetAsync(scratch, 0, 256, s);
    if (e != hipSuccess) return (int)e;
    if (io & 1) hipLaunchKernelGGL(absmax_bf16_kernel, dim3((unsigned)min((ng + 255) / 256, 4096L)), dim3(256), 0, s, (const __bf16*)gout, ng, amax);
    else hipLaunchKernelGGL(absmax_kernel, dim3((unsigned)min((ng + 255) / 256, 4096L)), dim3(256), 0, s, (const float*)gout, ng, amax);
    const Steps stp = make_steps(D, H, W);
    typedef void (*tile_t)(const float*, const float*, const unsigned*, const unsigned*, const unsigned*, const unsigned*, float*, int, int,
                           int, long, long, int, int, int, int, int, int, Steps);
    static const tile_t tiles[2][4] = {
        {splat_binned_tile_kernel<LF_MAP_O2C, 0>, splat_binned_tile_kernel<LF_MAP_O2C, 1>, splat_binned_tile_kernel<LF_MAP_O2C, 2>,
         splat_binned_tile_kernel<LF_MAP_O2C, 3>},
        {splat_binned_tile_kernel<LF_MAP_C2O, 0>, splat_binned_tile_kernel<LF_MAP_C2O, 1>, splat_binned_tile_kernel<LF_MAP_C2O, 2>,
         splat_binned_tile_kernel<LF_MAP_C2O, 3>}};
    static const tile_t tiles16[2][4] = {
        {splat_binned_tile16_kernel<LF_MAP_O2C, 0>, splat_binned_tile16_kernel<LF_MAP_O2C, 1>, splat_binned_tile16_kernel<LF_MAP_O2C, 2>,
         splat_binned_tile16_kernel<LF_MAP_O2C, 3>},
        {splat_binned_tile16_kernel<LF_MAP_C2O, 0>, splat_binned_tile16_kernel<LF_MAP_C2O, 1>, splat_binned_tile16_kernel<LF_MAP_C2O, 2>,
         splat_binned_tile16_kernel<LF_MAP_C2O, 3>}};
    for (int n0 = 0; n0 < N; n0 += cv) {
      const int m = min(cv, N - n0);
      e = hipMemsetAsync(cnt, 0, (size_t)2 * cv * nt * 4, s);
      if (e != hipSuccess) return (int)e;
      const dim3 gbin((unsigned)(((long)((W + 3) / 4) * ((H + 3) / 4) * ((D + 3) / 4) + 3) / 4), (unsigned)m);
      if (kind == LF_MAP_O2C) {
        hipLaunchKernelGGL((splat_bin_kernel<LF_MAP_O2C, false>), gbin, dim3(256), 0, s, coef, cnt, off, list, n0, nvox, cap, (int)nt, ntx, nty, D, H, W, stp);
// ... 44 lines not shown
```

latentfusion_amd/engine.py:

```python
import collections
import contextlib
import math

import torch

from . import _lib, ops
from ._lib import LF_EPI_LRELU, LF_EPI_PIXELNORM, LF_MAP_O2C, check

NCOEF = 24
NPAR = 10


def _s():
    return torch.cuda.current_stream().cuda_stream


class _CameraCoefs(torch.autograd.Function):

    @staticmethod
    def forward(ctx, params, intr, cube, z_span, h, w):
        L = _lib.lib()
        n = params.shape[0]
        coefs = torch.empty(n, NCOEF, device=params.device, dtype=torch.float32)
        jac = torch.empty(n, NCOEF, NPAR, device=params.device, dtype=torch.float32)
        check(L.lf_camera_coefs(params.contiguous().data_ptr(), intr.contiguous().data_ptr(), cube, z_span, h, w,
                                coefs.data_ptr(), jac.data_ptr(), n, _s()), 'lf_camera_coefs')
        ctx.save_for_backward(jac)
        return coefs

    @staticmethod
    def backward(ctx, g):
        L = _lib.lib()
        jac, = ctx.saved_tensors
        n = jac.shape[0]
        gp = torch.empty(n, NPAR, device=jac.device, dtype=torch.float32)
        check(L.lf_camera_coefs_bwd(g.contiguous().data_ptr(), jac.data_ptr(), gp.data_ptr(), n, _s()), 'lf_camera_coefs_bwd')
        return gp, None, None, None, None, None


def camera_params(camera):
    return torch.cat((camera.log_quaternion, camera.translation, camera.viewport), dim=1)


def camera_intrinsics(camera):
    K = camera.intrinsic
    return torch.stack((K[:, 0, 0], K[:, 1, 1], K[:, 0, 2], K[:, 1, 2]), dim=1).contiguous()


def camera_coefs(camera, cube_size, crop_h, crop_w):
    return _CameraCoefs.apply(camera_params(camera), camera_intrinsics(camera), float(cube_size), float(camera.z_span),
                              int(crop_h), int(crop_w))


def _pose_loss_fwd(lg, cf, tdepth, tmask, weights, H, W, masked=False, tn=None):
    L = _lib.lib()
    N, _, h, w = lg.shape
    nbytes = L.lf_pose_loss_scratch_bytes(N, h, w, H, W)
    scratch = torch.empty(nbytes // 4 + 1, device=lg.device, dtype=torch.float32)
    sums = torch.empty(N, 8, device=lg.device, dtype=torch.float32)
    losses = torch.empty(N, 8, device=lg.device, dtype=torch.float32)
    gsums = torch.empty(N, 8, device=lg.device, dtype=torch.float32)
    a = (lg.data_ptr(), cf.data_ptr(), tdepth.data_ptr(), tmask.data_ptr(), weights.data_ptr(), sums.data_ptr(), losses.data_ptr())
    b = (scratch.data_ptr(), scratch.numel() * 4, N) + (tn or ()) + (h, w, H, W, _s())
    if masked and tn is None:
        check(L.lf_pose_loss_fwd_masked(*a, *b), 'lf_pose_loss_fwd_masked')
    elif masked:
        check(L.lf_pose_loss_fwd_masked_mt(*a, *b), 'lf_pose_loss_fwd_masked_mt')
    elif tn is None:
        check(L.lf_pose_loss_fwd(*a, gsums.data_ptr(), *b), 'lf_pose_loss_fwd')
    else:
        check(L.lf_pose_loss_fwd_mt(*a, gsums.data_ptr(), *b), 'lf_pose_loss_fwd_mt')
    return losses, gsums, scratch


def _pose_loss_bwd(lg, cf, tdepth, tmask, gsums, glogits, gcoefs, scratch, H, W, tn=None):
    L = _lib.lib()
    N, _, h, w = lg.shape
    a = (lg.data_ptr(), cf.data_ptr(), tdepth.data_ptr(), tmask.data_ptr(), gsums.data_ptr(), glogits.data_ptr(), gcoefs.data_ptr(),
         scratch.data_ptr(), scratch.numel() * 4, N) + (tn or ()) + (h, w, H, W, _s())
    if tn is None:
        check(L.lf_pose_loss_bwd(*a), 'lf_pose_loss_bwd')
    else:
        check(L.lf_pose_loss_bwd_mt(*a), 'lf_pose_loss_bwd_mt')


class _PoseLoss(torch.autograd.Function):

    @staticmethod
    def forward(ctx, logits, coefs, tdepth, tmask, weights, H, W, tn=None):
        lg = ops.cl(logits)
        cf = coefs.detach().contiguous()
        losses, gsums, scratch = _pose_loss_fwd(lg, cf, tdepth, tmask, weights, H, W, tn=tn)
        ctx.save_for_backward(lg, cf, tdepth, tmask, gsums, scratch)
        ctx.dims = (H, W, tn)
        ctx.mark_non_differentiable(losses)
        return losses[:, 4].clone(), losses

    @staticmethod
    def backward(ctx, g_total, _g_losses):
        lg, cf, tdepth, tmask, gsums, scratch = ctx.saved_tensors
        H, W, tn = ctx.dims
        gs = (gsums * (g_total * (tn[1] if tn is not None else lg.shape[0])).unsqueeze(1)).contiguous()
        glogits = torch.empty_like(lg)
        gcoefs = torch.zeros(lg.shape[0], NCOEF, device=lg.device, dtype=torch.float32)
        _pose_loss_bwd(lg, cf, tdepth, tmask, gs, glogits, gcoefs, scratch, H, W, tn)
        return glogits, gcoefs, None, None, None, None, None, None


def pose_loss(logits, coefs, tdepth, tmask, weights, H, W):
    return _PoseLoss.apply(logits, coefs, tdepth, tmask, weights, H, W)


@contextlib.contextmanager
def _frozen(params):
    live = [p for p in params if p.requires_grad]
    for p in live:
        p.requires_grad_(False)
    try:
        yield
    finally:
        for p in live:
            p.requires_grad_(True)


def _prev(i, acts, norms, flags):
    return (acts[i], norms[i - 1], flags) if i > 0 else None


class _CameraBlocks:
    folds_prev = wide = wino16 = plain_factor_only = False

    def __init__(self, convs, z):
        self.w = [c.module.weight for c in convs]
        self.bias = [c.bias for c in convs]
        self.he = [ops.he_constant(w) for w in self.w]
        self.dev = z.device

    def grad_bounds(self):
        return None


class _Fp32Direct(_CameraBlocks):

    def __init__(self, convs, z):
        super().__init__(convs, z)
        self.packs = [(ops.pack_conv3x3(w), ops.pack_conv3x3(w, transpose=True)) for w in self.w]
        self.folds_prev = _block_kinds([tuple(w.shape[:2]) for w in self.w], z.shape[1])[0]

    def forward(self, li, x, flags, depth_inner=False):
        return ops._conv3x3_raw(x, self.packs[li][0], self.bias[li], self.w[li].shape[0], self.he[li], flags, True)

    def data_grad(self, i, g, acts, norms, flags, bounds):
        if self.folds_prev:
            return ops.conv3x3_bwd_data(g, self.packs[i][1], self.w[i].shape[1], self.he[i], _prev(i, acts, norms, flags))
        gpre = ops._epilogue_bwd(g, acts[i + 1], norms[i], flags)
        return ops._conv3x3_raw(gpre, self.packs[i][1], None, self.w[i].shape[1], self.he[i], 0, False)[0]


class _Winograd16(_CameraBlocks):
    folds_prev = wino16 = True

    def __init__(self, convs, z):
        super().__init__(convs, z)
        self.packs = [(ops.pack_conv3d_c16_wino(w), ops.pack_conv3d_c16_wino(w, transpose=True)) for w in self.w]
        self.rider = None

    def ride_projection(self, proj_pack, proj_bias, proj_he):
        self.rider = (proj_pack, proj_bias, proj_he)

    def forward(self, li, x, flags, depth_inner=False):
        if self.rider is not None and li == len(self.w) - 1:
            return ops.conv3d_c16_wino_projfwd(x, self.packs[li][0], self.bias[li], self.he[li], flags, *self.rider, flags)
        return ops.conv3d_c16_wino(x, self.packs[li][0], self.bias[li], self.he[li], flags)

    def data_grad(self, i, g, acts, norms, flags, bounds):
        return ops.conv3d_c16_wino(g, self.packs[i][1], None, self.he[i], 0, prev=_prev(i, acts, norms, flags))[0]


class _Direct16F16x3(_CameraBlocks):
    folds_prev = plain_factor_only = True
    _pack, _conv = staticmethod(ops.pack_conv3d_c16_split), staticmethod(ops.conv3d_c16_split)

    def __init__(self, convs, z):
        super().__init__(convs, z)
        self.packs = [(self._pack(w), self._pack(w, transpose=True)) for w in self.w]
        self.x0_bound = None

    def grad_bounds(self):
        return ops.amax_buffer(None, self.dev, rows=len(self.w) + 1)

    def forward(self, li, x, flags, depth_inner=False):
        return self._conv(x, self.packs[li][0], self.bias[li], self.he[li], flags, amax_in=self.x0_bound if li == 0 else None)

    def data_grad(self, i, g, acts, norms, flags, bounds):
        return self._conv(g, self.packs[i][1], None, self.he[i], 0, prev=_prev(i, acts, norms, flags), amax_in=bounds[i + 1],
                          amax_out=bounds[i])[0]


class _WideWinograd(_CameraBlocks):
    wide = True

    def forward(self, li, x, flags, depth_inner=False):
        return ops.wide_conv(x, self.w[li], self.bias[li], self.he[li], flags, depth_inner=depth_inner)

    def data_grad(self, i, g, acts, norms, flags, bounds):
        gpre = ops._epilogue_bwd(g, acts[i + 1], norms[i], flags)
        return ops.wide_conv(gpre, self.w[i], None, self.he[i], 0, transpose=True)[0]


class _WideWinogradF16x3(_CameraBlocks):
    wide = plain_factor_only = True

    def __init__(self, convs, z):
        super().__init__(convs, z)
        self.x_bound = [ops.amax_buffer(z.abs().amax(), self.dev)] + [
            ops.amax_buffer(torch.tensor(math.sqrt(w.shape[1])), self.dev) for w in self.w[1:]]
        for w in self.w:
            ops._pk(w, 'wxf', lambda w_: ops.pack_conv_wino_fused_f16x3(w_))
            ops._pk(w, 'wxb', lambda w_: ops.pack_conv_wino_fused_f16x3(w_, transpose=True))

    def forward(self, li, x, flags, depth_inner=False):
        return ops.wide_conv_f16x3(x, self.w[li], self.bias[li], self.he[li], flags, depth_inner=depth_inner, amax_in=self.x_bound[li])

    def data_grad(self, i, g, acts, norms, flags, bounds):
        amax = ops.amax_buffer(None, self.dev)
        gpre = ops.epilogue_bwd_amax(g, acts[i + 1], norms[i], flags, amax)
        return ops.wide_conv_f16x3(gpre, self.w[i], None, self.he[i], 0, transpose=True, amax_in=amax)[0]


CONV_MODES = ('auto', 'fp32', 'winograd', 'f16x3')


def _block_kinds(shapes, C):
    c16 = C == 16 and len(shapes) > 0 and all(tuple(sh) == (16, 16) for sh in shapes)
    wide = len(shapes) > 0 and all(co >= 64 and ci >= 64 and co % 4 == 0 and ci % 4 == 0 for co, ci in shapes)
    return c16, wide


def select_camera_blocks(conv_mode, shapes, C):
    if conv_mode not in CONV_MODES:
        raise ValueError(conv_mode)
    c16, wide = _block_kinds(shapes, C)
    if conv_mode == 'auto':
        conv_mode = 'winograd' if (c16 or wide) else 'fp32'
    if conv_mode == 'f16x3' and not (c16 or wide):
        raise NotImplementedError('f16x3 mode is implemented for 16->16 and wide (>= 64 channel) camera blocks')
    if conv_mode == 'winograd' and not (c16 or wide):
        raise NotImplementedError('winograd mode needs 16->16 or wide (>= 64 channel) camera blocks')
    if conv_mode == 'fp32':
        return conv_mode, _Fp32Direct
    if conv_mode == 'winograd':
        return conv_mode, _Winograd16 if c16 else _WideWinograd
    return conv_mode, _Direct16F16x3 if c16 else _WideWinogradF16x3


_Tail = collections.namedtuple('_Tail', 'zp pnorm feat leaf occ_saved')


class RenderLoopEngine:

    LOSS_KEYS = ('depth', 'ov_depth', 'iou', 'mask')
    EXPLICIT_DECODER = True
    EXPLICIT_OCCLUSION = True
    PROJ_GEMM = True

    @staticmethod
    def supports(photographer, loss_weights):
        return (photographer.projection_type in ('factor', 'sum')
                and not photographer.skip_connections
                and all(b.interpolate is None for b in photographer.camera_blocks)
                and photographer.predict_depth and photographer.predict_mask and not photographer.predict_color
                and photographer.camera_config[-1] % 4 == 0)

    CONV_MODES = CONV_MODES
    FUSE_FORMS = ('fwd',)
    _select_blocks = staticmethod(select_camera_blocks)

    def __init__(self, photographer, z_obj, target_obs, loss_weights, conv_mode='auto', fuse_projection=None):
        self.ph = photographer
        self.cube = photographer.cube_size
        dev = z_obj.device
        self.z = self._resident_volume(photographer, z_obj)
        self.S = self.z.shape[-1]
        self.C = self.z.shape[1]
        self.crop = photographer.out_size
        self.tdepth = target_obs.depth.reshape(-1).float().to(dev).contiguous()
        self.tmask = target_obs.mask.reshape(-1).float().to(dev).contiguous()
        self.H, self.W = target_obs.depth.shape[-2:]
        self.set_weights(loss_weights)
        convs = [conv for blk in photographer.camera_blocks for conv in (blk.conv1, blk.conv2)]
        self.nconv = len(convs)
        self.conv_mode, family = self._select_blocks(conv_mode, [tuple(c.module.weight.shape[:2]) for c in convs], self.C)
        self.generic_tail = photographer.projection_type != 'factor' or photographer.occlusion_module is not None
        if self.generic_tail and family.plain_factor_only:
            raise NotImplementedError("the split-precision conv modes drive the plain 'factor' renderer only")
        self.plan = family(convs, self.z)
        C, D = (convs[-1].module.weight.shape[0] if convs else self.C), self.S
        self.Cl = C
        self.occ = None
        if photographer.occlusion_module is not None and self.plan.wino16 and C == 16 and RenderLoopEngine.EXPLICIT_OCCLUSION:
            self.occ = self._plan_occlusion(photographer.occlusion_module)
        cout, pw = C, None
        self.proj = None
        if photographer.projection_type == 'factor':
            pw = photographer.projection_block.conv.module.weight
            cout = pw.shape[0]
            self.proj_rows_t = pw.detach().reshape(cout, C, D).permute(2, 1, 0).reshape(D * C, cout).contiguous()
            self.proj = (pw, photographer.projection_block.conv.bias, ops.he_constant(pw),
                         ops.pack_conv1x1(pw.reshape(cout, C, D).permute(0, 2, 1).reshape(cout, D * C)),
                         ops.pack_conv1x1(pw.reshape(cout, C, D).permute(2, 1, 0).reshape(D * C, cout)))
        can_fuse = self.plan.wino16 and cout == 16 and C == 16 and not self.generic_tail
        if fuse_projection is None:
            fuse_projection = ('fwd',) if can_fuse else ()
        elif fuse_projection is False:
            fuse_projection = ()
        elif fuse_projection is True:
            fuse_projection = self.FUSE_FORMS
        if any(f not in self.FUSE_FORMS for f in fuse_projection):
            raise ValueError(f'fuse_projection {fuse_projection!r}: this engine fuses {self.FUSE_FORMS}')
        if fuse_projection and not can_fuse:
            raise NotImplementedError("fuse_projection needs conv_mode 'winograd' on 16-channel blocks and a 16-channel projection")
        self.fuse_projection = tuple(fuse_projection)
        self.proj_fused = None
        if self.fuse_projection:
            wdm = pw.reshape(cout, C, D).permute(0, 2, 1).reshape(cout, D * C)
            self.proj_fused = (ops.pack_wino_proj(wdm), ops.pack_wino_proj(wdm, transpose=True))
        if 'fwd' in self.fuse_projection:
            self.plan.ride_projection(self.proj_fused[0], self.proj[1], self.proj[2])
        self._wide_factor = self.plan.wide and not self.generic_tail
        self.dev = dev
        self._params = list(photographer.parameters())
        self._intr = None
        self.heads = None
        obs = list(photographer.output_blocks)
        if len(obs) > 1 and all(getattr(ob, 'activation', None) is None and getattr(ob.conv, 'kernel_size', 0) == 1
                                and ob.conv.bias is not None for ob in obs):
            self.heads = (torch.cat([ob.conv.module.weight.detach() for ob in obs], dim=0).contiguous(),
                          torch.cat([ob.conv.bias.detach() for ob in obs], dim=0).contiguous())
        self.dec = None
        dec = photographer.image_decoder
        blocks2d = list(dec.down_blocks) + list(dec.up_blocks)
        plain = (dec.input_block is None and dec.output_block is None and self.heads is not None
                 and (not self.generic_tail or (self.occ is not None and photographer.projection_type == 'factor'))
                 and (len(dec.up_blocks) < 2 or len(dec.down_blocks) < 2)
                 and all(getattr(b, 'interpolate', True) is None for b in blocks2d) and len(blocks2d) > 0
                 and all(c.module.weight.dim() == 4 and tuple(c.module.weight.shape[2:]) == (3, 3) and c.module.weight.shape[0] <= 64
                         for b in blocks2d for c in (b.conv1, b.conv2)))
        if plain and RenderLoopEngine.EXPLICIT_DECODER:
            self.dec = []
            for blk in blocks2d:
                for conv in (blk.conv1, blk.conv2):
                    w = conv.module.weight
                    self.dec.append((w, conv.bias, ops.he_constant(w), ops.pack_conv3x3(w), ops.pack_conv3x3(w, transpose=True)))
            hw = self.heads[0]
            self.heads_pack = (ops.he_constant(hw), ops.pack_conv1x1(hw.reshape(hw.shape[0], hw.shape[1])),
                               ops.pack_conv1x1(hw.reshape(hw.shape[0], hw.shape[1]).t()))

    @staticmethod
    def _resident_volume(photographer, z_obj):
        z = ops.cl(z_obj.reshape(1, *z_obj.shape[-4:]))
        if len(photographer.object_blocks):
            with torch.no_grad():
                zo = z
                for blk in photographer.object_blocks:
                    zo = blk(zo)
            z = ops.cl(zo.detach())
        return z

    def set_weights(self, loss_weights):
        self.weights = torch.tensor([loss_weights.get(k, 0.0) for k in self.LOSS_KEYS], dtype=torch.float32,
                                    device=self.z.device)
        self.w_latent = float(loss_weights.get('latent', 0.0))

    def forward_backward(self, camera, need_grad=True, z_target_latent=None, params=None, masked_depth=False):
        if masked_depth and need_grad:
            raise ValueError('masked_depth is the forward-only loss form of the ranking estimators (no gradient is defined here)')
        if self.w_latent != 0.0 and z_target_latent is None:
            raise ValueError("the loss weights carry a 'latent' term: pass z_target_latent (LatentFusionModel.compute_latent_code)")
        params = (camera_params(camera) if params is None else params).detach().contiguous()
        K = camera.intrinsic
        if self._intr is None or self._intr[0] is not K or self._intr[1] != K._version:
            self._intr = (K, K._version, camera_intrinsics(camera))
        intr = self._intr[2]
        n = params.shape[0]
        zt = z_target_latent if (z_target_latent is not None and self.w_latent != 0.0) else None
        if zt is not None and zt.shape[0] == 1 and n > 1:
            zt = zt.expand(n, *zt.shape[1:])
        with _frozen(self._params):
            return self._run(params, intr, float(camera.z_span), need_grad, zt, masked_depth)

    def _run(self, params, intr, z_span, need_grad, zt, masked_depth):
        return self._forward_backward_group(params, intr, z_span, need_grad, 1.0, zt, masked_depth)

    @staticmethod
    def _plan_occlusion(om):
        from .modules.blocks import OutputBlock
        blocks = list(om.down_blocks) + list(om.up_blocks)
        ib, ob = om.input_block, om.output_block
        if (ib is None or not isinstance(ob, OutputBlock) or ob.activation is not None or len(om.down_blocks) != 1
                or len(om.up_blocks) != 1 or any(b.interpolate is not None for b in blocks)):
            return None
        w1, wo = ib.conv.module.weight, ob.conv.module.weight
        convs = [c for b in blocks for c in (b.conv1, b.conv2)]
        shapes = [tuple(c.module.weight.shape) for c in convs]
        if (tuple(w1.shape) != (17, 17, 1, 1, 1) or tuple(wo.shape) != (1, 16, 1, 1, 1) or shapes[0] != (16, 17, 3, 3, 3)
                or any(sh != (16, 16, 3, 3, 3) for sh in shapes[1:]) or ib.conv.bias is None or ob.conv.bias is None):
            return None
        dev = w1.device
        wi = torch.zeros(17, 20, device=dev, dtype=torch.float32)
        wi[:, :17] = w1.detach().reshape(17, 17) * ops.he_constant(w1)
        bi = torch.zeros(20, device=dev, dtype=torch.float32)
        bi[:17] = ib.conv.bias.detach()
        w2 = convs[0].module.weight.detach()
        w2a = w2[:, :16].contiguous()
        he2 = ops.he_constant(w2)
        w27 = (w2[:, 16].reshape(16, 27).t() * he2).float().contiguous()
        pk = ops.pack_conv3d_c16_wino
        first = (convs[0].bias, he2, pk(w2a), pk(w2a, transpose=True), w27)
        rest = [(c.bias, ops.he_constant(c.module.weight), pk(c.module.weight), pk(c.module.weight, transpose=True)) for c in convs[1:]]
        wo2 = wo.detach().reshape(1, 16)
        head = (ob.conv.bias, ops.he_constant(wo), ops.pack_conv1x1(wo2))
        return dict(wi=wi.contiguous(), bi=bi, first=first, rest=rest, head=head, head_w16=wo2.reshape(16).float().contiguous())

    def _occlusion_fwd(self, zc, flags):
        L = _lib.lib()
        o, s, dev = self.occ, _s(), self.dev
        n, _, D, H, W = zc.shape
        P = H * W
        ta, t16 = ops.empty_cl(zc.shape, dev), torch.empty(n, 1, D, H, W, device=dev, dtype=torch.float32)
        with ops._timed('occ_input_fwd'):
            check(L.lf_occ_input_fwd(zc.data_ptr(), o['wi'].data_ptr(), o['bi'].data_ptr(), ta.data_ptr(), t16.data_ptr(), n, D, P,
                                     ops.SLOPE, s), 'lf_occ_input_fwd')
        b2, he2, pa, _pat, w27 = o['first']
        pre = ops.empty_cl(zc.shape, dev)
        with ops._timed('occ_conv17_fwd'):
            check(L.lf_occ_conv17_fwd(t16.data_ptr(), w27.data_ptr(), pre.data_ptr(), n, D, H, W, s), 'lf_occ_conv17_fwd')
        y, nrm = ops.conv3d_c16_wino(ta, pa, b2, he2, flags, prev=(pre, None, _lib.LF_EPI_ADD), out=pre)
        ys, ns = [y], [nrm]
        for (b, he, pk, _pkt) in o['rest']:
            y, nrm = ops.conv3d_c16_wino(ys[-1], pk, b, he, flags)
            ys.append(y)
            ns.append(nrm)
        hb, hhe, hpk = o['head']
        wocc = torch.empty(n, 1, D, H, W, device=dev, dtype=torch.float32)
        if D <= 256:
            with ops._timed('column_softmax_head'):
                check(L.lf_column_softmax_head_fwd(ys[-1].data_ptr(), o['head_w16'].data_ptr(), hb.data_ptr() if hb is not None else None,
                                                   hhe, wocc.data_ptr(), None, n, D, P, s), 'lf_column_softmax_head_fwd')
        else:
            logits = torch.empty(n, 1, D, H, W, device=dev, dtype=torch.float32)
            ops._conv1x1_raw(ys[-1], hpk, hb, n, D * P, 16, 1, D * P * 16, 0, 1, logits, hhe, 0)
            with ops._timed('column_softmax'):
                check(L.lf_column_softmax_fwd(logits.data_ptr(), wocc.data_ptr(), None, n, D, P, s), 'lf_column_softmax_fwd')
        if self.proj is not None:
            return None, (ta, t16, ys, ns, wocc)
        zs = ops.empty_cl(zc.shape, dev)
        check(L.lf_column_scale_fwd(zc.data_ptr(), wocc.data_ptr(), zs.data_ptr(), n * D * P, 16, s), 'lf_column_scale_fwd')
        return zs, (ta, t16, ys, ns, wocc)

    def _occlusion_bwd(self, g_zs, zc, saved, flags, prev, proj_bwd=None):
        L = _lib.lib()
        o, s, dev = self.occ, _s(), self.dev
        ta, t16, ys, ns, wocc = saved
        n, _, D, H, W = zc.shape
        P = H * W
        gl = torch.empty_like(wocc)
        if proj_bwd is not None and D <= 256:
            with ops._timed('occ_weight_grad_softmax_bwd'):
                check(L.lf_occ_weight_grad_softmax_bwd(zc.data_ptr(), proj_bwd[0].data_ptr(), proj_bwd[1].data_ptr(), proj_bwd[2], wocc.data_ptr(),
                                                       gl.data_ptr(), n, D, P, s), 'lf_occ_weight_grad_softmax_bwd')
        else:
            gw = torch.empty_like(wocc)
            if proj_bwd is not None:
                check(L.lf_occ_weight_grad(zc.data_ptr(), proj_bwd[0].data_ptr(), proj_bwd[1].data_ptr(), proj_bwd[2], gw.data_ptr(), n, D, P, s),
                      'lf_occ_weight_grad')
            else:
                check(L.lf_column_scale_bwd(g_zs.data_ptr(), zc.data_ptr(), wocc.data_ptr(), None, gw.data_ptr(), n * D * P, 16, s),
                      'lf_column_scale_bwd')
            check(L.lf_column_softmax_bwd(wocc.data_ptr(), gw.data_ptr(), None, gl.data_ptr(), n, D, P, s), 'lf_column_softmax_bwd')
        hhe = o['head'][1]
        g = ops.empty_cl(zc.shape, dev)
        with ops._timed('occ_head_bwd'):
            check(L.lf_occ_head_bwd(gl.data_ptr(), o['head_w16'].data_ptr(), hhe, ys[-1].data_ptr(), ns[-1].data_ptr(), flags, ops.SLOPE,
                                    g.data_ptr(), n * D * P, s), 'lf_occ_head_bwd')
        for i in range(len(o['rest']) - 1, -1, -1):
            _b, he, _pk, pkt = o['rest'][i]
            g = ops.conv3d_c16_wino(g, pkt, None, he, 0, prev=(ys[i], ns[i], flags))[0]
        _b2, he2, _pa, pat, w27 = o['first']
        gp16 = torch.empty_like(t16)
        gta = ops.conv3d_c16_wino(g, pat, None, he2, 0, prev=(ta, None, LF_EPI_LRELU))[0]
        with ops._timed('occ_conv17_bwd'):
            check(L.lf_occ_conv17_bwd(g.data_ptr(), t16.data_ptr(), w27.data_ptr(), gp16.data_ptr(), n, D, H, W, ops.SLOPE, s),
                  'lf_occ_conv17_bwd')
        gz = ops.empty_cl(zc.shape, dev)
        if proj_bwd is not None:
            gp2d, ppack_t, phe = proj_bwd
            with ops._timed('occ_input_bwd'):
                check(L.lf_occ_input_bwd_proj(gta.data_ptr(), gp16.data_ptr(), o['wi'].data_ptr(), gp2d.data_ptr(), ppack_t.data_ptr(), phe,
                                              wocc.data_ptr(), gz.data_ptr(), n, D, P, ops.SLOPE, zc.data_ptr(), prev[1].data_ptr(), prev[2], s),
                      'lf_occ_input_bwd_proj')
            return gz
        with ops._timed('occ_input_bwd'):
            check(L.lf_occ_input_bwd(gta.data_ptr(), None, gp16.data_ptr(), o['wi'].data_ptr(), g_zs.data_ptr(),
                                     wocc.data_ptr(), gz.data_ptr(), n * D * P, ops.SLOPE, zc.data_ptr(), prev[1].data_ptr(), prev[2], s),
                  'lf_occ_input_bwd')
        return gz

    def _forward_backward_group(self, params, intr, z_span, need_grad, grad_scale, zt=None, masked_depth=False):
        n = params.shape[0]
        flags = LF_EPI_LRELU | LF_EPI_PIXELNORM
        coefs, jac, cf20 = self._coefficients(params, intr, z_span, n)
        proj_gemm = self.PROJ_GEMM and self._wide_factor and not need_grad
        acts, norms, rode = self._blocks_fwd(self._resample(cf20, n), flags, proj_gemm)
        tail = self._tail_fwd(acts[-1], rode, flags, need_grad, proj_gemm, n)
        latent_grad = zt is not None and need_grad
        explicit = self.dec is not None and not latent_grad
        if explicit:
            dacts, dnorms, logits = self._decoder_fwd(tail.zp, tail.pnorm, flags, n)
        else:
            logits = self._decoder_autograd(tail.feat, need_grad)
        if latent_grad:
            cf_leaf = coefs.detach().requires_grad_(True)
            with torch.enable_grad():
                total, losses = self._loss_autograd(logits, cf_leaf)
                lat = self._latent_distance(tail.feat, zt, n)
                total = total + self.w_latent * lat
                losses = losses.clone()
                losses[:, 5] = lat.detach()
                losses[:, 4] += self.w_latent * lat.detach()
                objective = self._objective(total)
            g_leaf, g_cf = torch.autograd.grad(objective, [tail.leaf, cf_leaf])
            gp = None
        else:
            lg = ops.cl(logits.detach())
            losses, gsums, scratch = self._loss_fwd(lg, coefs, masked_depth)
            if not need_grad:
                if zt is not None:
                    lat = self._latent_distance(tail.zp, zt, n)
                    losses[:, 5] = lat
                    losses[:, 4] += self.w_latent * lat
                return losses, None
            glogits = torch.empty_like(lg)
            g_cf = torch.empty(n, NCOEF, device=self.dev, dtype=torch.float32)
            self._loss_bwd(lg, coefs, gsums, glogits, g_cf, scratch)
            if explicit:
                gp, g_leaf = self._decoder_bwd(glogits, dacts, dnorms, flags, n), None
            else:
                gp, (g_leaf,) = None, torch.autograd.grad(logits, [tail.leaf], grad_outputs=[glogits])
        g, first, bounds = self._tail_bwd(tail, gp, g_leaf, acts, norms, flags, n)
        for i in range(first, -1, -1):
            g = self.plan.data_grad(i, g, acts, norms, flags, bounds)
        return self._finish_backward(g, g_cf, cf20, jac, n, grad_scale, losses)

    def _coefficients(self, params, intr, z_span, n):
        L = _lib.lib()
        params = params.contiguous()
        intr = intr.contiguous()
        coefs = torch.empty(n, NCOEF, device=self.dev, dtype=torch.float32)
        jac = torch.empty(n, NCOEF, NPAR, device=self.dev, dtype=torch.float32)
        check(L.lf_camera_coefs(params.data_ptr(), intr.data_ptr(), float(self.cube), z_span, self.crop,
                                self.crop, coefs.data_ptr(), jac.data_ptr(), n, _s()), 'lf_camera_coefs')
        cf20 = torch.empty(n, 20, device=self.dev, dtype=torch.float32)
        cf20[:, :18] = coefs[:, :18]
        return coefs, jac, cf20

    def _resample(self, cf20, n):
        L = _lib.lib()
        S = self.S
        x0 = ops.empty_cl((n, self.C, S, S, S), self.dev)
        with ops._timed('resample_fwd'):
            check(L.lf_resample3d_fwd(self.z.data_ptr(), 1, cf20.data_ptr(), LF_MAP_O2C, x0.data_ptr(), n, S, S, S, self.C, _s()),
                  'lf_resample3d_fwd')
        return x0

    def _blocks_fwd(self, x0, flags, proj_gemm):
        acts, norms, rode = [x0], [], []
        last = self.nconv - 1
        for li in range(self.nconv):
            y, nrm, *rode = self.plan.forward(li, acts[-1], flags, depth_inner=proj_gemm and li == last)
            acts.append(y)
            norms.append(nrm)
        return acts, norms, rode

    def _tail_fwd(self, act, rode, flags, need_grad, proj_gemm, n):
        if self.occ is not None:
            return self._occlusion_tail_fwd(act, flags, need_grad, n)
        if self.generic_tail:
            return self._module_tail_fwd(act, need_grad)
        return self._factor_fwd(act, rode, flags, need_grad, proj_gemm, n)

    def _tail_bwd(self, tail, gp, g_leaf, acts, norms, flags, n):
        if self.occ is not None:
            return self._occlusion_tail_bwd(tail, gp, g_leaf, acts, norms, flags, n)
        if self.generic_tail:
            return self._module_tail_bwd(tail, g_leaf, acts, norms, flags)
        return self._factor_bwd(tail, gp, g_leaf, acts, norms, flags, n)

    def _proj_pre_grad(self, tail, gp, g_leaf, flags):
        return gp if gp is not None else ops._epilogue_bwd(ops.cl(g_leaf), tail.zp, tail.pnorm, flags)

    def _factor_fwd(self, act, rode, flags, need_grad, proj_gemm, n):
        L = _lib.lib()
        pw, pb, phe, ppack, _ppack_t = self.proj
        cout, S, Cl = pw.shape[0], self.S, self.Cl
        if rode:
            zp, pnorm = rode
        elif proj_gemm:
            with ops._timed('factor_project_fwd'):
                x2 = act.view(n * S * S, S * Cl)
                if pb is not None:
                    rows = torch.addmm(pb.detach(), x2, self.proj_rows_t, alpha=phe)
                else:
                    rows = torch.mm(x2, self.proj_rows_t).mul_(phe)
                torch.nn.functional.leaky_relu_(rows, ops.SLOPE)
                pnorm = torch.empty(n * S * S, device=self.dev, dtype=torch.float32)
                check(L.lf_pixelnorm_fwd(rows.data_ptr(), rows.data_ptr(), pnorm.data_ptr(), n * S * S, cout, ops.PN_EPS, _s()), 'lf_pixelnorm_fwd')
            zp = rows.view(n, S, S, cout).permute(0, 3, 1, 2)
        else:
            zp = ops.empty_cl((n, cout, S, S), self.dev)
            with ops._timed('factor_project_fwd'):
                pnorm = ops._conv1x1_raw(act, ppack, pb, n, S * S, Cl, S, S * S * S * Cl, S * S * Cl, cout, zp, phe, flags)
        leaf = zp.detach().requires_grad_(need_grad)
        return _Tail(zp, pnorm, leaf, leaf, None)

    def _factor_bwd(self, tail, gp, g_leaf, acts, norms, flags, n):
        L = _lib.lib()
        pw, _pb, phe, _ppack, ppack_t = self.proj
        cout, S, Cl, nconv = pw.shape[0], self.S, self.Cl, self.nconv
        gp = self._proj_pre_grad(tail, gp, g_leaf, flags)
        fused = self._proj_bwd_fused(gp, acts, norms, flags) if self.plan.folds_prev else None
        if fused is not None:
            return fused + (None,)
        g = ops.empty_cl((n, Cl, S, S, S), self.dev)
        bounds = self.plan.grad_bounds()
        if self.plan.folds_prev:
            with ops._timed('factor_project_bwd'):
                check(L.lf_conv1x1_bwd_data(gp.data_ptr(), ppack_t.data_ptr(), g.data_ptr(), n, S * S, cout, S * Cl,
                                            S * S * S * Cl, Cl, Cl, S * S * Cl, phe, acts[nconv].data_ptr(),
                                            norms[nconv - 1].data_ptr(), flags, ops.SLOPE,
                                            bounds[nconv].data_ptr() if bounds is not None else None, _s()), 'lf_conv1x1_bwd_data')
        else:
            ops._conv1x1_raw(gp, ppack_t, None, n, S * S, cout, 1, S * S * cout, 0, S * Cl, g, phe, 0,
                             yaddr=(S * S * S * Cl, Cl, Cl, S * S * Cl))
        return g, nconv - 1, bounds

    def _proj_bwd_fused(self, gp, acts, norms, flags):
        return None

    def _occlusion_tail_fwd(self, act, flags, need_grad, n):
        zs, occ_saved = self._occlusion_fwd(act, flags)
        if self.proj is None:
            leaf = zs.detach().requires_grad_(need_grad)
            with torch.set_grad_enabled(need_grad):
                zp = ops.column_sum(leaf)
            return _Tail(zp, None, zp, leaf, occ_saved)
        pw, pb, phe, ppack, _ppack_t = self.proj
        cout, S, Cl = pw.shape[0], self.S, self.Cl
        zp = ops.empty_cl((n, cout, S, S), self.dev)
        with ops._timed('factor_project_fwd'):
            pnorm = ops._conv1x1_raw(act, ppack, pb, n, S * S, Cl, S, S * S * S * Cl, S * S * Cl, cout, zp, phe, flags,
                                     xscale=occ_saved[4])
        leaf = zp.detach().requires_grad_(need_grad)
        return _Tail(zp, pnorm, leaf, leaf, occ_saved)

    def _occlusion_tail_bwd(self, tail, gp, g_leaf, acts, norms, flags, n):
        S, Cl, nconv = self.S, self.Cl, self.nconv
        proj_bwd = None
        if self.proj is None:
            g_zs = ops.cl(g_leaf)
        else:
            pw, _pb, phe, _ppack, ppack_t = self.proj
            cout = pw.shape[0]
            gp = self._proj_pre_grad(tail, gp, g_leaf, flags)
            with ops._timed('factor_project_bwd'):
                if Cl == 16 and cout == 16 and (S * S) % 16 == 0:
                    g_zs, proj_bwd = None, (gp, ppack_t, phe)
                else:
                    g_zs = ops.empty_cl((n, Cl, S, S, S), self.dev)
                    ops._conv1x1_raw(gp, ppack_t, None, n, S * S, cout, 1, S * S * cout, 0, S * Cl, g_zs, phe, 0,
                                     yaddr=(S * S * S * Cl, Cl, Cl, S * S * Cl))
        g = self._occlusion_bwd(g_zs, acts[-1], tail.occ_saved, flags, (acts[nconv], norms[nconv - 1], flags), proj_bwd)
        return g, nconv - 1, None

    def _module_tail_fwd(self, act, need_grad):
        from .recon.utils import get_normalized_voxel_depth
        leaf = act.detach().requires_grad_(need_grad)
        with torch.set_grad_enabled(need_grad):
            zt_ = leaf
            if self.ph.occlusion_module is not None:
                occ = self.ph.occlusion_module(torch.cat((zt_, get_normalized_voxel_depth(zt_)), dim=1))
                wocc = ops.column_softmax(occ)[0]
                if tuple(occ.shape[-3:]) != tuple(zt_.shape[-3:]):
                    wocc = ops.column_softmax(ops.resize_nearest_to(occ, zt_.size(-1)))[0]
                zt_ = ops.column_scale(zt_, wocc)
            zp = ops.column_sum(zt_) if self.ph.projection_type == 'sum' else self.ph.projection_block(zt_)
        return _Tail(zp, None, zp, leaf, None)

    def _module_tail_bwd(self, tail, g_leaf, acts, norms, flags):
        g = ops.cl(g_leaf)
        if self.plan.folds_prev:
            g = ops._epilogue_bwd(g, acts[self.nconv], norms[self.nconv - 1], flags)
        return g, self.nconv - 1, None

    def _decoder_fwd(self, zp, pnorm, flags, n):
        dacts, dnorms = [zp], [pnorm]
        for (w2, b2, he2, pk2, _pkt2) in self.dec:
            y2, n2 = ops._conv3x3_raw(dacts[-1], pk2, b2, w2.shape[0], he2, flags, True)
            dacts.append(y2)
            dnorms.append(n2)
        hw, hb = self.heads
        hhe, hpk, _hpkt = self.heads_pack
        hh, ww = dacts[-1].shape[-2:]
        logits = ops.empty_cl((n, hw.shape[0], hh, ww), self.dev)
        ops._conv1x1_raw(dacts[-1], hpk, hb, n, hh * ww, hw.shape[1], 1, hh * ww * hw.shape[1], 0, hw.shape[0], logits, hhe, 0)
        return dacts, dnorms, logits

    def _decoder_bwd(self, glogits, dacts, dnorms, flags, n):
        L = _lib.lib()
        hw = self.heads[0]
        cin_h = hw.shape[1]
        hh, ww = dacts[-1].shape[-2:]
        g2 = ops.empty_cl((n, cin_h, hh, ww), self.dev)
        fuse_h = cin_h == 16
        check(L.lf_conv1x1_bwd_data(glogits.data_ptr(), self.heads_pack[2].data_ptr(), g2.data_ptr(), n, hh * ww, hw.shape[0],
                                    cin_h, hh * ww * cin_h, cin_h, cin_h if fuse_h else (1 << 30), 0, self.heads_pack[0],
                                    dacts[-1].data_ptr() if fuse_h else None, dnorms[-1].data_ptr() if fuse_h else None,
                                    flags if fuse_h else 0, ops.SLOPE, None, _s()), 'lf_conv1x1_bwd_data')
        if not fuse_h:
            g2 = ops._epilogue_bwd(g2, dacts[-1], dnorms[-1], flags)
        for i in range(len(self.dec) - 1, -1, -1):
            w2, _b2, he2, _pk2, pkt2 = self.dec[i]
            cin2 = w2.shape[1]
            if cin2 in (16, 32, 64):
                g2 = ops.conv3x3_bwd_data(g2, pkt2, cin2, he2, (dacts[i], dnorms[i], flags))
            else:
                g2 = ops._epilogue_bwd(ops.conv3x3_bwd_data(g2, pkt2, cin2, he2, None), dacts[i], dnorms[i], flags)
        return g2

    def _decoder_autograd(self, feat, need_grad):
        with torch.set_grad_enabled(need_grad), ops.wide2d_f16x3(self.conv_mode == 'f16x3'):
            yimg, rescale = self.ph.decode_features(feat)
            if self.heads is not None:
                logits = ops.conv1x1(yimg, self.heads[0], self.heads[1])
            else:
                logits = torch.cat([ob(yimg) for ob in self.ph.output_blocks], dim=1)
            return rescale(logits) if rescale is not None else logits

    def _loss_fwd(self, lg, coefs, masked_depth):
        return _pose_loss_fwd(lg, coefs, self.tdepth, self.tmask, self.weights, self.H, self.W, masked_depth)

    def _loss_bwd(self, lg, coefs, gsums, glogits, g_cf, scratch):
        _pose_loss_bwd(lg, coefs, self.tdepth, self.tmask, gsums, glogits, g_cf, scratch, self.H, self.W)

    def _loss_autograd(self, logits, coefs):
        return pose_loss(logits, coefs, self.tdepth, self.tmask, self.weights, self.H, self.W)

    def _objective(self, total):
        return total.mean()

    def _latent_distance(self, zp, zt, n):
        return 1.0 - torch.cosine_similarity(zp.reshape(n, -1), zt.reshape(n, -1).to(zp.dtype), 1, 1e-8)

    def _bwd_coef(self, g, cf20, gcoef18, n):
        L = _lib.lib()
        S = self.S
        nbytes = L.lf_resample3d_bwd_coef_scratch_bytes(n, S, S, S)
        scratch = torch.empty(nbytes // 4 + 1, device=self.dev, dtype=torch.float32)
        with ops._timed('resample_bwd_coef'):
            check(L.lf_resample3d_bwd_coef(g.data_ptr(), self.z.data_ptr(), 1, cf20.data_ptr(), gcoef18.data_ptr(),
                                           scratch.data_ptr(), scratch.numel() * 4, n, S, S, S, self.C, _s()), 'lf_resample3d_bwd_coef')

    def _finish_backward(self, g, g_cf, cf20, jac, n, grad_scale, losses):
        L = _lib.lib()
        dev, s = self.dev, _s()
        gcoef18 = torch.empty(n, 18, device=dev, dtype=torch.float32)
        self._bwd_coef(g, cf20, gcoef18, n)
        gcoefs = g_cf.contiguous()
        gcoefs[:, :18] = gcoef18
        gparams = torch.empty(n, NPAR, device=dev, dtype=torch.float32)
        check(L.lf_camera_coefs_bwd(gcoefs.data_ptr(), jac.data_ptr(), gparams.data_ptr(), n, s), 'lf_camera_coefs_bwd')
        if grad_scale != 1.0:
            gparams *= grad_scale
        return losses, gparams
```

latentfusion_amd/engine_multi.py:

```python
import torch

from . import _lib, ops
from ._lib import check
from .engine import LF_MAP_O2C, RenderLoopEngine, _PoseLoss, _pose_loss_bwd, _pose_loss_fwd, _s


def distinct_volumes(z_objs):
    vols, index, seen = [], [], {}
    for z in z_objs:
        k = seen.get(id(z))
        if k is None:
            k = seen[id(z)] = len(vols)
            vols.append(z)
        index.append(k)
    return vols, index


def check_volumes(z_objs, num_targets):
    z_objs = list(z_objs)
    if len(z_objs) != num_targets:
        raise ValueError(f'{len(z_objs)} volumes for {num_targets} targets: a volume list holds one entry per target')
    for i, z in enumerate(z_objs):
        if not isinstance(z, torch.Tensor):
            raise ValueError(f'volume {i} is a {type(z).__name__}: expected a tensor')
        if z.dim() < 4:
            raise ValueError(f'volume {i} has shape {tuple(z.shape)}: expected (.., C, S, S, S)')
    kinds = {(tuple(z.shape[-4:]), z.dtype, z.device) for z in z_objs}
    if len(kinds) != 1:
        raise ValueError('the volumes differ in shape, dtype or device: ' + ', '.join(
            f'{shape} {dtype} {dev}' for shape, dtype, dev in sorted(kinds, key=str)))
    return z_objs


class MultiTargetEngine(RenderLoopEngine):

    MAX_ROWS = 65535

    def __init__(self, photographer, z_obj, targets, loss_weights, conv_mode='auto', fuse_projection=None):
        targets = list(targets)
        if not targets:
            raise ValueError('MultiTargetEngine needs at least one target')
        for i, t in enumerate(targets):
            if len(t) != 1:
                raise ValueError(f'target {i} holds {len(t)} frames: every target is one single-frame Observation')
        sizes = {tuple(t.depth.shape[-2:]) for t in targets}
        if len(sizes) != 1:
            raise ValueError(f'the targets differ in frame size: {sorted(sizes)}')
        if conv_mode not in RenderLoopEngine.CONV_MODES:
            raise NotImplementedError(f'conv_mode {conv_mode!r}: the multi-target engine runs {RenderLoopEngine.CONV_MODES}')
        if fuse_projection is True or (isinstance(fuse_projection, (tuple, list, set)) and 'bwd' in fuse_projection):
            raise NotImplementedError('the fused projection backward is an experimental.RenderLoopEngineX option')
        vols = index = None
        if isinstance(z_obj, (list, tuple)):
            vols, index = distinct_volumes(check_volumes(z_obj, len(targets)))
            z_obj = vols[0]
        super().__init__(photographer, z_obj, targets[0], loss_weights, conv_mode=conv_mode, fuse_projection=fuse_projection)
        dev = self.dev
        self.zs = self.vol_of = None
        if vols is not None:
            self.zs = ops.cl(torch.cat([self.z] + [self._resident_volume(photographer, z) for z in vols[1:]]))
            self.z = self.zs[:1]
            self.vol_of = index
            self._tables = {}
        self.tdepth = torch.stack([t.depth.reshape(-1).float().to(dev) for t in targets]).contiguous()
        self.tmask = torch.stack([t.mask.reshape(-1).float().to(dev) for t in targets]).contiguous()
        self.T = len(targets)
        self._n = None
        self._max_batch = self.MAX_ROWS

    def max_batch(self):
        return self._max_batch

    def set_streams(self, k):
        raise NotImplementedError('hypothesis groups on several streams are an experimental.RenderLoopEngineX option')

    def forward_backward_graph(self, camera, params):
        raise NotImplementedError('hipGraph replay is an experimental.RenderLoopEngineX option')

    def forward_backward(self, camera, n, need_grad=True, z_target_latent=None, params=None, masked_depth=False):
        n = int(n)
        N = len(camera) if params is None else params.shape[0]
        if n < 1 or N != self.T * n:
            raise ValueError(f'{N} hypotheses are not {self.T} targets x n = {n}')
        if N > self._max_batch:
            raise ValueError(f'{N} rows exceed the largest batch this renderer can launch ({self._max_batch}): '
                             'split the targets into smaller groups')
        if z_target_latent is not None and z_target_latent.shape[0] != N:
            if z_target_latent.shape[0] != self.T:
                raise ValueError(f'z_target_latent has {z_target_latent.shape[0]} rows: expected {N} or {self.T}')
            z_target_latent = z_target_latent.repeat_interleave(n, dim=0)
        self._n = n
        try:
            return RenderLoopEngine.forward_backward(self, camera, need_grad, z_target_latent, params, masked_depth)
        finally:
            self._n = None

    def _loss_fwd(self, lg, coefs, masked_depth):
        return _pose_loss_fwd(lg, coefs, self.tdepth, self.tmask, self.weights, self.H, self.W, masked_depth, (self.T, self._n))

    def _loss_bwd(self, lg, coefs, gsums, glogits, g_cf, scratch):
        _pose_loss_bwd(lg, coefs, self.tdepth, self.tmask, gsums, glogits, g_cf, scratch, self.H, self.W, (self.T, self._n))

    def _loss_autograd(self, logits, coefs):
        return _PoseLoss.apply(logits, coefs, self.tdepth, self.tmask, self.weights, self.H, self.W, (self.T, self._n))

    def _objective(self, total):
        return total.view(self.T, self._n).mean(dim=1).sum()

    def _latent_distance(self, zp, zt, n):
        k = self._n
        return torch.cat([RenderLoopEngine._latent_distance(self, zp[t * k:(t + 1) * k], zt[t * k:(t + 1) * k], k)
                          for t in range(self.T)])

    def _table(self, rows):
        n = self._n
        if rows != self.T * n:
            raise ValueError(f'{rows} rows are not {self.T} targets x n = {n}')
        if n not in self._tables:
            self._tables[n] = ops.volume_table([k for k in self.vol_of for _ in range(n)], self.zs.shape[0], self.dev)
        return self._tables[n]

    def _resample(self, cf20, n):
        if self.zs is None:
            return RenderLoopEngine._resample(self, cf20, n)
        L = _lib.lib()
        S = self.S
        x0 = ops.empty_cl((n, self.C, S, S, S), self.dev)
        table = self._table(n)
        with ops._timed('resample_fwd'):
            check(L.lf_resample3d_fwd_indexed(self.zs.data_ptr(), self.zs.shape[0], table.data_ptr(), cf20.data_ptr(), LF_MAP_O2C,
                                              x0.data_ptr(), n, S, S, S, self.C, _s()), 'lf_resample3d_fwd_indexed')
        return x0

    def _bwd_coef(self, g, cf20, gcoef18, n):
        L = _lib.lib()
        S = self.S
        if self.zs is None:
            name, vol = 'lf_resample3d_bwd_coef_part', (self.z.data_ptr(), 1)
        else:
            name, vol = 'lf_resample3d_bwd_coef_indexed', (self.zs.data_ptr(), self.zs.shape[0], self._table(n).data_ptr())
        nbytes = getattr(L, name + '_scratch_bytes')(n, self._n, S, S, S)
        scratch = torch.empty(nbytes // 4 + 1, device=self.dev, dtype=torch.float32)
        with ops._timed('resample_bwd_coef'):
            check(getattr(L, name)(g.data_ptr(), *vol, cf20.data_ptr(), gcoef18.data_ptr(), scratch.data_ptr(), scratch.numel() * 4,
                                   n, S, S, S, self.C, self._n, _s()), name)
```

latentfusion_amd/pose/estimation.py:

```python
import contextlib
import copy
import math
from collections import defaultdict
from pathlib import Path

import torch

from .. import three
from ..modules.geometry import Camera
from ..utils import ExponentialScheduler, LinearScheduler
from . import utils as pu
from .loss import default_pose_loss, weigh_losses

DEFAULT_TRANSLATION_STD = 0.01
DEFAULT_QUATERION_STD = 10.0 / 180.0 * math.pi


def _load_toml(path):
    import tomli
    with open(path, 'rb') as f:
        return tomli.load(f)


def load_from_config(config, model, **kwargs):
# ... 389 lines not shown
        self.converge_threshold, self.converge_patience = converge_threshold, converge_patience
        self.loss_schedules = dict(loss_schedules) if loss_schedules else {}
        self.track_stats = track_stats

    def _estimate(self, z_obj, target_obs, **kwargs):
        if 'camera' in kwargs:
            camera = kwargs['camera']
        else:
            camera = pu.sample_cameras_with_estimate(n=self.num_samples, camera_est=self.initial_pose(target_obs))
        target_obs = target_obs.to(self.device)
        camera = camera.zoom(None, self.model.input_size, self.model.camera_dist).to(self.device)
        camera = self._sync_cameras_from_rank0(camera)
        ranking = []
        stats, history = self._optimize_camera(z_obj, target_obs, camera, iters=self.num_iters, ranking=ranking)
        best = Camera.cat([c for c, _, _ in ranking])
        if self.track_stats and self.return_camera_history:
            return best, stats, history
        if self.track_stats:
            return best, stats
        if self.return_camera_history:
            return best, history
        return best

    def loss_and_grad(self, z_obj, target_obs, cameras, step=0, z_target_latent=None):
        z_depth, z_mask_logits, z_pred_latent = self._render_observation(z_obj, cameras)
        optim_weights = copy.copy(self.loss_weights)
        optim_weights.update({k: v.get(step) for k, v in self.loss_schedules.items()})
        loss_dict = self.loss_func(target_obs, z_depth, z_mask_logits, cameras, z_pred_latent=z_pred_latent,
                                   z_target_latent=z_target_latent)
        optim_loss = sum(weigh_losses(loss_dict, optim_weights).values())
        optim_loss.mean().backward()
        rank_loss = sum(weigh_losses(loss_dict, self.loss_weights).values()).detach()
        return loss_dict, optim_loss.detach(), rank_loss, optim_weights

    def _engine_for(self, z_obj, target_obs, schedules=()):
        eng = super()._engine_for(z_obj, target_obs, schedules=self.loss_schedules)
        if eng is not None and self.engine_streams > 1:
            eng.set_streams(self.engine_streams)
        return eng

    @classmethod
    def get_optimizer(cls, name, *args, **kwargs):
        from torch import optim
        table = {'adamw': optim.AdamW, 'adam': optim.Adam, 'sgd': optim.SGD, 'adagrad': optim.Adagrad}
        if name not in table:
            raise ValueError(f'Unknow optimizer {name!r}')
        return table[name](*args, **kwargs)

    def start(self, z_obj, target_obs, cameras, ranking=None):
        rank, size = self._sharding()
        shard, full_cpu = None, None
        if size > 1:
            from .. import parallel
            b, e = parallel.shard_range(len(cameras), rank, size)
            if e <= b:
                raise ValueError(f'shard_hypotheses: {len(cameras)} hypotheses cannot be split over {size} ranks')
            shard, full_cpu = (b, e, len(cameras)), cameras.to('cpu')
            cameras = cameras[b:e]
        st = self._start_local(z_obj, target_obs, cameras, ranking)
        st['shard'], st['template_full_cpu'] = shard, full_cpu
        return st

    def _start_local(self, z_obj, target_obs, cameras, ranking):
        engine = self._engine_for(z_obj, target_obs)
        if engine is not None:
            from ..engine import camera_params
            P = camera_params(cameras).detach().clone().contiguous()
            P.requires_grad_(True)
            cam = cameras._like(log_quaternion=P[:, 0:3], translation=P[:, 3:6], viewport=P[:, 6:10])
            return {
                'engine': engine, 'P': P, 'z_obj': z_obj, 'target': target_obs, 'cam': cam, 'params': [P],
                'opt': BatchedOptimizer(self.optimizer, [P]),
                'sched': _PlateauLR(len(cameras), self.learning_rate, self.lr_reduce_patience,
                                    self.lr_reduce_threshold, self.lr_reduce_factor),
                'ranking': [] if ranking is None else ranking, 'step': 0, 'converge_count': 0,
                'stat_history': {}, 'camera_history': [], 'target_q': target_obs.camera.quaternion,
                'template_cpu': cameras.to('cpu'),
            }
        cam = pu.parameterize_camera(cameras, optimize_viewport=True)
        params = [cam.log_quaternion, cam.translation, cam.viewport]
        return {
            'z_obj': z_obj, 'target': target_obs, 'cam': cam, 'params': params,
            'opt': BatchedOptimizer(self.optimizer, params),
            'sched': _PlateauLR(len(cameras), self.learning_rate, self.lr_reduce_patience, self.lr_reduce_threshold,
                                self.lr_reduce_factor),
            'ranking': [] if ranking is None else ranking, 'step': 0, 'converge_count': 0,
            'stat_history': {}, 'camera_history': [], 'target_q': target_obs.camera.quaternion,
        }

    def iterate(self, st):
        with self._frozen_model():
            return self._iterate_engine(st) if 'engine' in st else self._iterate_modules(st)

    def _iterate_modules(self, st):
        cam, params, target_obs, step = st['cam'], st['params'], st['target'], st['step']
        for p in params:
            p.grad = None
        z_target_latent = None
        if self.loss_weights.get('latent', 0.0) > 0.0:
            with torch.no_grad():
                z_target_latent = self.model.compute_latent_code(target_obs, cam)
        loss_dict, optim_loss, rank_loss, optim_weights = self.loss_and_grad(st['z_obj'], target_obs, cam, step,
                                                                           z_target_latent)
        shard = st.get('shard')
        if shard is not None:
            from .. import parallel
            rows = torch.cat((rank_loss.unsqueeze(1), cam.log_quaternion.detach(), cam.translation.detach()), dim=1)
            rows = parallel.gather_rows(rows.contiguous(), shard[2]).cpu()
            rank_all = rows[:, 0].tolist()
            rank_host = rank_all[shard[0]:shard[1]]
            detached_all = st['template_full_cpu']._like(log_quaternion=rows[:, 1:4].clone(), translation=rows[:, 4:7].clone(),
                                                         viewport=None)
            if self.return_camera_history:
                st['camera_history'].append((rows[:, 0].clone(), detached_all))
            delta = self._track_best_items(st['ranking'], step, list(detached_all), rank_all)
            detached = cam.uncrop().detach().clone()
        else:
            rank_host = rank_loss.tolist()
            detached = cam.uncrop().detach().clone()
            if self.return_camera_history:
                st['camera_history'].append((rank_loss.cpu(), detached.to('cpu')))
            delta = self._track_best_items(st['ranking'], step, list(detached.to('cpu')), rank_host)
        if self.track_stats:
            angle = three.quaternion.angular_distance(detached.quaternion, st['target_q']).squeeze()
            trans = torch.norm(detached.translation - target_obs.camera.translation, dim=1).squeeze()
            self._record_stat_dict(st['stat_history'], {
                **{f'{k}_loss': v.detach().cpu() for k, v in loss_dict.items()},
                **{f'{k}_weight': v for k, v in optim_weights.items()},
                'delta': delta, 'converge_count': st['converge_count'], 'angle_dist': angle.cpu(),
                'trans_dist': trans.cpu(), 'optim_loss': optim_loss.cpu(), 'rank_loss': rank_loss.cpu()})
        st['opt'].step(st['sched'].lr)
        st['sched'].step(rank_host)
        if delta < self.converge_threshold:
            st['converge_count'] += 1
        elif delta > self.converge_threshold:
            st['converge_count'] = 0
        st['step'] += 1
        return st['converge_count'] >= self.converge_patience

    def _engine_weights(self, st, step):
        optim_weights = copy.copy(self.loss_weights)
        if self.loss_schedules:
            optim_weights.update({k: v.get(step) for k, v in self.loss_schedules.items()})
            st['engine'].set_weights(optim_weights)
        return optim_weights

    def _engine_launch(self, st, step):
        eng, P = st['engine'], st['P']
        optim_weights = self._engine_weights(st, step)
        with torch.no_grad():
            z_target_latent = None
            if optim_weights.get('latent', 0.0) != 0.0 or self.loss_weights.get('latent', 0.0) != 0.0:
                z_target_latent = self.model.compute_latent_code(st['target'], st['cam'])
            if self.engine_graph and z_target_latent is None and not self.loss_schedules and hasattr(eng, 'forward_backward_graph'):
                losses, gparams = eng.forward_backward_graph(st['cam'], P)
            else:
                losses, gparams = eng.forward_backward(st['cam'], need_grad=True, z_target_latent=z_target_latent, params=P)
            dev = torch.cat((losses[:, :6], P.detach()), dim=1)
            if st.get('shard') is not None:
                from .. import parallel
                dev = parallel.gather_rows(dev.contiguous(), st['shard'][2])
        slot = st.setdefault('pinned', {})
        key = step & 1
        if key not in slot or slot[key].shape != dev.shape:
            slot[key] = torch.empty(dev.shape, dtype=dev.dtype, pin_memory=True)
        slot[key].copy_(dev, non_blocking=True)
        ev = torch.cuda.Event()
        ev.record()
        return {'step': step, 'gparams': gparams, 'host': slot[key], 'event': ev, 'weights': optim_weights}

    def _iterate_engine(self, st):
        eng, P, step, target_obs = st['engine'], st['P'], st['step'], st['target']
        cur = st.pop('inflight', None)
        if cur is None or cur['step'] != step:
            cur = self._engine_launch(st, step)
        P.grad = cur['gparams']
        st['opt'].step(st['sched'].lr)
        if st.get('max_steps') is None or step + 1 < st['max_steps']:
            st['inflight'] = self._engine_launch(st, step + 1)
        cur['event'].synchronize()
        host = cur['host'].clone()
        optim_weights = cur['weights']
        comp = {k: host[:, i] for i, k in enumerate(eng.LOSS_KEYS)}
        if self.loss_weights.get('latent', 0.0) != 0.0 or 'latent' in self.loss_schedules:
            comp['latent'] = host[:, 5]
        rank = sum(self.loss_weights.get(k, 0.0) * v for k, v in comp.items())
        rank_host = rank.tolist()
        shard = st.get('shard')
        tpl = st['template_cpu'] if shard is None else st['template_full_cpu']
        detached = tpl._like(log_quaternion=host[:, 6:9].clone(), translation=host[:, 9:12].clone(), viewport=None)
        if self.return_camera_history:
            st['camera_history'].append((rank.clone(), detached))
        delta = self._track_best_items(st['ranking'], step, list(detached), rank_host)
        if self.track_stats:
            angle = three.quaternion.angular_distance(detached.quaternion, st['target_q'].cpu()).squeeze()
            trans = torch.norm(detached.translation - target_obs.camera.translation.cpu(), dim=1).squeeze()
            self._record_stat_dict(st['stat_history'], {
                **{f'{k}_loss': v for k, v in comp.items()}, **{f'{k}_weight': v for k, v in optim_weights.items()},
                'delta': delta, 'converge_count': st['converge_count'], 'angle_dist': angle, 'trans_dist': trans,
                'optim_loss': host[:, 4].clone(), 'rank_loss': rank.clone()})
        st['sched'].step(rank_host if shard is None else rank_host[shard[0]:shard[1]])
        if delta < self.converge_threshold:
            st['converge_count'] += 1
        elif delta > self.converge_threshold:
            st['converge_count'] = 0
        st['step'] += 1
        return st['converge_count'] >= self.converge_patience

    def _optimize_camera(self, z_obj, target_obs, cameras, iters, ranking):
        st = self.start(z_obj, target_obs, cameras, ranking)
        st['max_steps'] = iters
        for _ in range(iters):
            if self.iterate(st):
                break
        return st['stat_history'], st['camera_history']

    def estimate_batch(self, z_obj, targets, cameras=None):
        targets = list(targets)
        if not targets:
            raise ValueError('estimate_batch needs at least one target')
        for i, t in enumerate(targets):
            if len(t) != 1:
                raise ValueError(f'target {i} holds {len(t)} observations: the pose is estimated for one frame per target')
        sizes = {tuple(t.depth.shape[-2:]) for t in targets}
        if len(sizes) != 1:
            raise ValueError(f'the targets differ in frame size: {sorted(sizes)}')
        if cameras is not None:
            cameras = list(cameras)
            if len(cameras) != len(targets):
                raise ValueError(f'{len(cameras)} camera batches for {len(targets)} targets')
            counts = {len(c) for c in cameras}
            if len(counts) != 1:
                raise ValueError(f'every target needs the same number of hypotheses, got {sorted(counts)}')
        z_of = None
        if isinstance(z_obj, (list, tuple)):
            from ..engine_multi import check_volumes
            z_of = check_volumes(z_obj, len(targets))
        if self.shard_hypotheses:
            raise NotImplementedError('estimate_batch does not shard hypotheses over ranks')
        if cameras is None:
            cameras = [pu.sample_cameras_with_estimate(n=self.num_samples, camera_est=self.initial_pose(t)) for t in targets]
        if not self._multi_engine_applies(z_obj if z_of is None else z_of[0]):
            self.last_batch_groups = [1] * len(targets)
            return [self.estimate(z_obj if z_of is None else z_of[i], t, camera=c)
                    for i, (t, c) in enumerate(zip(targets, cameras))]
        if self.engine_streams > 1 or self.engine_graph:
            raise NotImplementedError('engine_streams / engine_graph are experimental.RenderLoopEngineX options')
        from ..engine_multi import MultiTargetEngine
        groups = self._batch_groups(len(targets), len(cameras[0]))
        try:
            with self._frozen_model():
                zoomed = [c.zoom(None, self.model.input_size, self.model.camera_dist).to(self.device) for c in cameras]
                if len({float(c.z_span) for c in zoomed}) != 1:
                    raise ValueError("the targets' cameras differ in z_span")
                dev_targets = [t.to(self.device) for t in targets]
                self.last_batch_groups = [e - b for b, e in groups]
                out = []
                for b, e in groups:
                    eng = MultiTargetEngine(self.model.photographer, z_obj if z_of is None else z_of[b:e], dev_targets[b:e],
                                            self.loss_weights,
                                            conv_mode=self.conv_mode, fuse_projection=self.fuse_projection)
                    out += self._run_batch(eng, dev_targets[b:e], zoomed[b:e])
                    del eng
                return out
        finally:
            self._engine_cache = None

    @staticmethod
    def _batch_groups(T, n):
        from ..engine_multi import MultiTargetEngine
        per = min(T, MultiTargetEngine.MAX_ROWS // n)
        if per < 1:
            raise ValueError(f'{n} hypotheses per target exceed the {MultiTargetEngine.MAX_ROWS} rows one render loop can carry')
        return [(b, min(T, b + per)) for b in range(0, T, per)]

    def _multi_engine_applies(self, z_obj):
        if not self.use_engine or self.loss_func is not default_pose_loss or not z_obj.is_cuda:
            return False
        from ..engine import RenderLoopEngine
        ph = getattr(self.model, 'photographer', None)
        if ph is None or not RenderLoopEngine.supports(ph, self.loss_weights):
            return False
        return all(k in RenderLoopEngine.LOSS_KEYS + ('latent',) for k in self.loss_schedules)

    def _batch_launch(self, st, step):
        eng, P, n = st['engine'], st['P'], st['n']
        optim_weights = self._engine_weights(st, step)
        with torch.no_grad():
            zt = None
            if optim_weights.get('latent', 0.0) != 0.0 or self.loss_weights.get('latent', 0.0) != 0.0:
                codes = [self.model.compute_latent_code(tg, c) for tg, c in zip(st['targets'], st['cam_t'])]
                zt = torch.cat([z.expand(n, *z.shape[1:]) if z.shape[0] == 1 else z for z in codes])
            losses, gparams = eng.forward_backward(st['cam'], n, need_grad=True, z_target_latent=zt, params=P)
            dev = torch.cat((losses[:, :6], P.detach()), dim=1)
        slot = st.setdefault('pinned', {})
        key = step & 1
        if key not in slot or slot[key].shape != dev.shape:
            slot[key] = torch.empty(dev.shape, dtype=dev.dtype, pin_memory=True)
        slot[key].copy_(dev, non_blocking=True)
        ev = torch.cuda.Event()
        ev.record()
        return {'step': step, 'gparams': gparams, 'host': slot[key], 'event': ev, 'weights': optim_weights}

    def _run_batch(self, eng, targets, zoomed):
        from ..engine import camera_params
        T, n = len(targets), len(zoomed[0])
        P = torch.cat([camera_params(c) for c in zoomed]).detach().clone().contiguous()
        P.requires_grad_(True)
        cam = Camera.cat(zoomed)._like(log_quaternion=P[:, 0:3], translation=P[:, 3:6], viewport=P[:, 6:10])
        st = {'engine': eng, 'P': P, 'n': n, 'cam': cam, 'targets': targets,
              'cam_t': [cam[t * n:(t + 1) * n] for t in range(T)]}
# ... 75 lines not shown
```

Before: 187.5.

## Stream projection backward and fuse coefficient-gradient finish with readback row packing

```diff
diff --git a/include/lf_hip.h b/include/lf_hip.h
--- a/include/lf_hip.h
+++ b/include/lf_hip.h
@@ -38,6 +38,9 @@
 int lf_resample3d_bwd_coef_part(const float* gout, const float* vol, int vol_n, const float* coef,
                                 float* gcoef, void* scratch, size_t scratch_bytes,
                                 int N, int D, int H, int W, int C, int part_n, void* stream);
+int lf_resample3d_bwd_coef_partials(const float* gout, const float* vol, int vol_n, const float* coef,
+                                    void* scratch, size_t scratch_bytes,
+                                    int N, int D, int H, int W, int C, int* nblk, void* stream);
 
 int lf_resample3d_fwd_indexed(const float* vol, int vol_n, const int32_t* vol_idx, const float* coef, int kind,
                               float* out, int N, int D, int H, int W, int C, void* stream);
@@ -76,6 +79,8 @@
                         long y_batch_stride, int y_row_stride, int y_slice_channels, long y_slice_stride,
                         float he, const float* prev_y, const float* prev_norm, unsigned prev_flags,
                         float slope, float* amax_out, void* stream);
+int lf_proj16_bwd_f32(const float* gp, const float* wpack_t, float* g, const float* act, const float* norm,
+                      int N, int D, long P, float he, unsigned flags, float slope, void* stream);
 
 #define LF_AMAX_FLOATS 2048
 size_t lf_conv3d_c16_split_wpack_halfs(void);
@@ -271,6 +276,8 @@
 int lf_camera_coefs(const float* params, const float* intrinsics, float cube_size, float z_span,
                     int crop_h, int crop_w, float* coefs, float* jac, int N, void* stream);
 int lf_camera_coefs_bwd(const float* gcoefs, const float* jac, float* gparams, int N, void* stream);
+int lf_coef_grad_finish(const float* partial, int nblk, const float* gcoefs, const float* jac, float* gparams,
+                        float grad_scale, const float* losses, const float* params, float* rows, int N, void* stream);
 
 size_t lf_pose_loss_scratch_bytes(int N, int h, int w, int H, int W);
 int lf_pose_loss_fwd(const float* logits, const float* coefs, const float* target_depth,
diff --git a/latentfusion_amd/_lib.py b/latentfusion_amd/_lib.py
--- a/latentfusion_amd/_lib.py
+++ b/latentfusion_amd/_lib.py
@@ -26,6 +26,7 @@
     'lf_resample3d_fwd': (c_int, [P, c_int, P, c_int, P, c_int, c_int, c_int, c_int, c_int, P]),
     'lf_resample3d_bwd_coef_scratch_bytes': (c_size_t, [c_int, c_int, c_int, c_int]),
     'lf_resample3d_bwd_coef': (c_int, [P, P, c_int, P, P, P, c_size_t, c_int, c_int, c_int, c_int, c_int, P]),
+    'lf_resample3d_bwd_coef_partials': (c_int, [P, P, c_int, P, P, c_size_t, c_int, c_int, c_int, c_int, c_int, P, P]),
     'lf_resample3d_bwd_coef_part_scratch_bytes': (c_size_t, [c_int, c_int, c_int, c_int, c_int]),
     'lf_resample3d_bwd_coef_part': (c_int, [P, P, c_int, P, P, P, c_size_t, c_int, c_int, c_int, c_int, c_int, c_int, P]),
     'lf_resample3d_fwd_indexed': (c_int, [P, c_int, P, P, c_int, P, c_int, c_int, c_int, c_int, c_int, P]),
@@ -45,6 +46,7 @@
                                     c_float, P]),
     'lf_conv1x1_bwd_data': (c_int, [P, P, P, c_int, c_int, c_int, c_int, c_long, c_int, c_int, c_long, c_float, P, P,
                                     c_uint, c_float, P, P]),
+    'lf_proj16_bwd_f32': (c_int, [P, P, P, P, P, c_int, c_int, c_long, c_float, c_uint, c_float, P]),
     'lf_conv3d_c16_split_wpack_halfs': (c_size_t, []),
     'lf_conv3d_c16_split_pairs': (None, [P]),
     'lf_conv3d_c16_split': (c_int, [P, P, P, P, P, c_int, c_int, c_int, c_int, c_float, c_uint, c_float, c_float, P, P,
@@ -136,6 +138,7 @@
     'lf_resize_bwd': (c_int, [P, P, c_int, c_int, c_int, c_int, c_int, c_int, c_int, c_int, P]),
     'lf_camera_coefs': (c_int, [P, P, c_float, c_float, c_int, c_int, P, P, c_int, P]),
     'lf_camera_coefs_bwd': (c_int, [P, P, P, c_int, P]),
+    'lf_coef_grad_finish': (c_int, [P, c_int, P, P, P, c_float, P, P, P, c_int, P]),
     'lf_pose_loss_scratch_bytes': (c_size_t, [c_int, c_int, c_int, c_int, c_int]),
     'lf_pose_loss_fwd': (c_int, [P, P, P, P, P, P, P, P, P, c_size_t, c_int, c_int, c_int, c_int, c_int, P]),
     'lf_pose_loss_bwd': (c_int, [P, P, P, P, P, P, P, P, c_size_t, c_int, c_int, c_int, c_int, c_int, P]),
diff --git a/latentfusion_amd/csrc/build.py b/latentfusion_amd/csrc/build.py
--- a/latentfusion_amd/csrc/build.py
+++ b/latentfusion_amd/csrc/build.py
@@ -3,9 +3,9 @@
 import sys
 
 HERE = os.path.dirname(os.path.abspath(__file__))
-SOURCES = ['resample.hip', 'conv.hip', 'pointwise.hip', 'image.hip', 'optim.hip', 'resize.hip', 'conv_split.hip', 'conv_wino.hip', 'wgrad.hip', 'sample2d.hip', 'gru.hip', 'wino_gemm.hip', 'reduce.hip', 'wino_fused.hip', 'conv_bf16.hip', 'occlusion.hip', 'conv_gru.hip', 'lift_mfma.hip', 'pw16.hip', 'wino_fused_f16x3.hip', 'wgrad_wide.hip']
+SOURCES = ['resample.hip', 'conv.hip', 'pointwise.hip', 'image.hip', 'optim.hip', 'resize.hip', 'conv_split.hip', 'conv_wino.hip', 'wgrad.hip', 'sample2d.hip', 'gru.hip', 'wino_gemm.hip', 'reduce.hip', 'wino_fused.hip', 'conv_bf16.hip', 'occlusion.hip', 'conv_gru.hip', 'lift_mfma.hip', 'pw16.hip', 'wino_fused_f16x3.hip', 'wgrad_wide.hip', 'proj_stream.hip', 'coef_finish.hip']
 LIB = os.path.join(HERE, 'liblf_hip.so')
-EXTRA = {'conv_split.hip': ['-fno-slp-vectorize'], 'conv_gru.hip': ['-fno-slp-vectorize']}
+EXTRA = {'conv_split.hip': ['-fno-slp-vectorize'], 'conv_gru.hip': ['-fno-slp-vectorize'], 'proj_stream.hip': ['-fno-slp-vectorize']}
 FLAGS = ['--offload-arch=gfx950', '-O3', '-std=c++17', '-fPIC', '-fno-gpu-rdc', '-Wall', '-Wno-unused-function']
 
 
diff --git a/latentfusion_amd/csrc/coef_finish.hip b/latentfusion_amd/csrc/coef_finish.hip
--- /dev/null
+++ b/latentfusion_amd/csrc/coef_finish.hip
@@ -0,0 +1,48 @@
+#include "lf_common.h"
+#include "resample_partials.h"
+
+namespace {
+
+constexpr int NP = 10;
+constexpr int NOUT = 24;
+constexpr int NROW = 16;
+static_assert(LF_COEF_PARTIAL == 18, "entries 0..17 of the coefficient block come from the resampler");
+
+__global__ void __launch_bounds__(256) coef_grad_finish_kernel(const float* __restrict__ partial, int nblk,
+                                                               const float* __restrict__ gtail, const float* __restrict__ jac,
+                                                               float* __restrict__ gparams, float grad_scale,
+                                                               const float* __restrict__ losses, const float* __restrict__ params,
+                                                               float* __restrict__ rows) {
+  const int n = blockIdx.x, t = threadIdx.x;
+  __shared__ double red[256];
+  __shared__ float gc[NOUT];
+  const double tot = lf_coef_partials_sum(partial, nblk, n, red);
+  if (t < LF_COEF_PARTIAL) gc[t] = (float)tot;
+  else if (t < NOUT) gc[t] = gtail[n * NOUT + t];
+  __syncthreads();
+  if (t < NP) {
+    double s = 0.0;
+    for (int j = 0; j < NOUT; ++j) s += (double)gc[j] * (double)jac[(n * NOUT + j) * NP + t];
+    float g = (float)s;
+    if (grad_scale != 1.0f) g *= grad_scale;
+    gparams[n * NP + t] = g;
+  }
+  if (rows != nullptr && t >= 64 && t < 64 + NROW) {
+    const int c = t - 64;
+    rows[n * NROW + c] = c < 6 ? losses[n * 8 + c] : params[n * NP + (c - 6)];
+  }
+}
+
+}
+
+extern "C" int lf_coef_grad_finish(const float* partial, int nblk, const float* gcoefs, const float* jac, float* gparams,
+                                   float grad_scale, const float* losses, const float* params, float* rows, int N,
+                                   void* stream) {
+  lf_clear_error();
+  if (!partial || !gcoefs || !jac || !gparams) return LF_EINVAL;
+  if (N <= 0 || nblk <= 0) return LF_EINVAL;
+  if (rows != nullptr && (!losses || !params)) return LF_EINVAL;
+  hipLaunchKernelGGL(coef_grad_finish_kernel, dim3(N), dim3(256), 0, (hipStream_t)stream, partial, nblk, gcoefs, jac, gparams,
+                     grad_scale, losses, params, rows);
+  return lf_launch_status();
+}
diff --git a/latentfusion_amd/csrc/lf_common.h b/latentfusion_amd/csrc/lf_common.h
--- a/latentfusion_amd/csrc/lf_common.h
+++ b/latentfusion_amd/csrc/lf_common.h
@@ -55,3 +55,4 @@
 
 int lf_internal_ring_bf16_set_wgs(int v);
 int lf_internal_fused_set_cfg(int v);
+int lf_internal_proj_stream_set_cfg(int v);
diff --git a/latentfusion_amd/csrc/proj_stream.hip b/latentfusion_amd/csrc/proj_stream.hip
--- /dev/null
+++ b/latentfusion_amd/csrc/proj_stream.hip
@@ -0,0 +1,119 @@
+#include "lf_common.h"
+
+namespace {
+
+int g_proj_stream_cfg = 1 * 4 + 1;
+
+template <int PF, unsigned FLAGS>
+__global__ void __launch_bounds__(256) proj16_bwd_stream_kernel(
+    const float* __restrict__ gp, const float* __restrict__ wpack_t, float* __restrict__ g,
+    const float* __restrict__ act, const float* __restrict__ norm,
+    int D, long P, float he, float slope, int stagger) {
+  constexpr bool FOLD = FLAGS != 0, PN = (FLAGS & LF_EPI_PIXELNORM) != 0;
+  const int lane = threadIdx.x & 63, wave = threadIdx.x >> 6;
+  const int li = lane & 15, cq = lane >> 4;
+  const int n = blockIdx.y;
+  const long p0 = (long)blockIdx.x * 64 + wave * 16;
+  if (p0 >= P) return;
+  const long p = p0 + li < P ? p0 + li : P - 1;
+
+  const f32x4 bfrag = *(const f32x4*)(gp + ((long)n * P + p) * 16 + cq * 4);
+  const float* wl = wpack_t + li * 16 + cq * 4;
+  const long vox0 = (long)n * D * P + p;
+  const long rec0 = vox0 * 16 + cq * 4;
+
+  unsigned first = 0;
+  if (stagger == 1) first = ((unsigned)blockIdx.x * 4u + (unsigned)wave + (unsigned)n) * 37u;
+  else if (stagger == 2) first = ((unsigned)blockIdx.x + (unsigned)n) * 37u;
+  const int d0 = __builtin_amdgcn_readfirstlane((int)(first % (unsigned)D));
+  auto depth = [&](int i) { const int d = d0 + i; return d >= D ? d - D : d; };
+
+  f32x4 wa[PF], ya[PF];
+  float na[PF];
+  auto request = [&](int u, int i) {
+    const int d = depth(i);
+    wa[u] = *(const f32x4*)(wl + (long)d * 256);
+    if (FOLD) ya[u] = __builtin_nontemporal_load((const f32x4*)(act + rec0 + (long)d * P * 16));
+    if (PN) na[u] = __builtin_nontemporal_load(norm + vox0 + (long)d * P);
+    __builtin_amdgcn_sched_barrier(0);
+  };
+  auto form = [&](const f32x4& w, const f32x4& yp, float nr, int d) {
+    f32x4 acc = (f32x4){0.f, 0.f, 0.f, 0.f};
+#pragma unroll
+    for (int st = 0; st < 4; ++st) acc = __builtin_amdgcn_mfma_f32_16x16x4f32(w[st], bfrag[st], acc, 0, 0, 0);
+    f32x4 v;
+#pragma unroll
+    for (int e = 0; e < 4; ++e) v[e] = __builtin_fmaf(acc[e], he, 0.f);
+    if (PN) {
+      float dot = __builtin_fmaf(v[3], yp[3], __builtin_fmaf(v[2], yp[2], __builtin_fmaf(v[0], yp[0], v[1] * yp[1])));
+      dot += __shfl_xor(dot, 16, 64);
+      dot += __shfl_xor(dot, 32, 64);
+      dot *= (1.f / 16.f);
+      const float rinv = 1.0f / nr;
+#pragma unroll
+      for (int e = 0; e < 4; ++e) v[e] = __builtin_fmaf(-yp[e], dot, v[e]) * rinv;
+    }
+    if (FLAGS & LF_EPI_LRELU) {
+#pragma unroll
+      for (int e = 0; e < 4; ++e) v[e] = yp[e] > 0.f ? v[e] : v[e] * slope;
+    }
+    __builtin_nontemporal_store(v, (f32x4*)(g + rec0 + (long)d * P * 16));
+  };
+
+  const int Dg = D - D % PF;
+  if (Dg > 0) {
+#pragma unroll
+    for (int u = 0; u < PF; ++u) request(u, u);
+    for (int i0 = 0; i0 < Dg; i0 += PF) {
+#pragma unroll
+      for (int u = 0; u < PF; ++u) {
+        const int i = i0 + u;
+        form(wa[u], ya[u], na[u], depth(i));
+        request(u, i + PF < D ? i + PF : D - 1);
+      }
+    }
+  }
+#pragma unroll
+  for (int u = 0; u < PF - 1; ++u)
+    if (Dg == 0 && u < D) request(u, u);
+#pragma unroll
+  for (int u = 0; u < PF - 1; ++u)
+    if (Dg + u < D) form(wa[u], ya[u], na[u], depth(Dg + u));
+}
+
+}
+
+int lf_internal_proj_stream_set_cfg(int v) {
+  const int prev = g_proj_stream_cfg;
+  if (v >= 0 && v < 12 && (v & 3) != 3) g_proj_stream_cfg = v;
+  return prev;
+}
+
+extern "C" int lf_proj16_bwd_f32(const float* gp, const float* wpack_t, float* g, const float* act, const float* norm,
+                                 int N, int D, long P, float he, unsigned flags, float slope, void* stream) {
+  lf_clear_error();
+  if (!gp || !wpack_t || !g) return LF_EINVAL;
+  if (N <= 0 || D <= 0 || P <= 0) return LF_EINVAL;
+  if (flags & ~(LF_EPI_LRELU | LF_EPI_PIXELNORM)) return LF_EINVAL;
+  if (flags != 0 && !act) return LF_EINVAL;
+  if ((flags & LF_EPI_PIXELNORM) && !norm) return LF_EINVAL;
+  if (!lf_aligned16(gp) || !lf_aligned16(wpack_t) || !lf_aligned16(g) || !lf_aligned16(act)) return LF_EALIGN;
+  if ((((uintptr_t)norm) & 3u) != 0) return LF_EALIGN;
+  const long gx = (P + 63) / 64;
+  if (gx > 0x7fffffffL || N > 65535 || (long)D * 256 > 0x7fffffffL) return LF_EINVAL;
+  const dim3 grid((unsigned)gx, (unsigned)N), block(256);
+  hipStream_t s = (hipStream_t)stream;
+  const int cfg = g_proj_stream_cfg, stagger = cfg & 3;
+#define LAUNCH(PF, F) hipLaunchKernelGGL((proj16_bwd_stream_kernel<PF, F>), grid, block, 0, s, gp, wpack_t, g, act, norm, D, P, \
+                                         he, slope, stagger)
+#define LAUNCH_F(PF) switch (flags) { case 0: LAUNCH(PF, 0u); break; case 1: LAUNCH(PF, 1u); break; \
+                                      case 2: LAUNCH(PF, 2u); break; default: LAUNCH(PF, 3u); break; }
+  switch (cfg >> 2) {
+    case 0: LAUNCH_F(2); break;
+    case 2: LAUNCH_F(8); break;
+    default: LAUNCH_F(4); break;
+  }
+#undef LAUNCH_F
+#undef LAUNCH
+  return lf_launch_status();
+}
diff --git a/latentfusion_amd/csrc/resample.hip b/latentfusion_amd/csrc/resample.hip
--- a/latentfusion_amd/csrc/resample.hip
+++ b/latentfusion_amd/csrc/resample.hip
@@ -1,4 +1,5 @@
 #include "lf_common.h"
+#include "resample_partials.h"
 #include <type_traits>
 
 namespace {
@@ -89,18 +90,8 @@
                                                                 int nblk, float* __restrict__ gcoef) {
   const int n = blockIdx.x;
   __shared__ double red[256];
-  const int comp = threadIdx.x % 18;
-  const int grp = threadIdx.x / 18;
-  double s = 0.0;
-  if (grp < 14)
-    for (int b = grp; b < nblk; b += 14) s += (double)partial[((long)n * nblk + b) * 18 + comp];
-  red[threadIdx.x] = (grp < 14) ? s : 0.0;
-  __syncthreads();
-  if (threadIdx.x < 18) {
-    double tot = 0.0;
-    for (int g = 0; g < 14; ++g) tot += red[g * 18 + threadIdx.x];
-    gcoef[(long)n * 18 + threadIdx.x] = (float)tot;
-  }
+  const double tot = lf_coef_partials_sum(partial, nblk, n, red);
+  if (threadIdx.x < LF_COEF_PARTIAL) gcoef[(long)n * LF_COEF_PARTIAL + threadIdx.x] = (float)tot;
 }
 
 template <int KIND>
@@ -969,13 +960,14 @@
 
 static int bwd_coef_finish(const float* partial, int nblk, float* gcoef, int N, hipStream_t s) {
   if (int e = lf_launch_status()) return e;
+  if (gcoef == nullptr) return 0;
   hipLaunchKernelGGL(resample_bwd_coef_reduce, dim3(N), dim3(256), 0, s, partial, nblk, gcoef);
   return lf_launch_status();
 }
 
 static int bwd_coef_launch(const float* gout, const float* vol, int vol_n, const float* coef,
                            float* gcoef, void* scratch, size_t scratch_bytes,
-                           int N, int part_n, int D, int H, int W, int C, void* stream) {
+                           int N, int part_n, int D, int H, int W, int C, void* stream, int* nblk_out = nullptr) {
   if (N <= 0 || D <= 0 || H <= 0 || W <= 0 || C <= 0) return LF_EINVAL;
   if (vol_n != 1 && vol_n != N) return LF_EINVAL;
   BwdCoefPlan p;
@@ -989,6 +981,7 @@
     if (nb * N > 0x7fffffffL) return LF_EINVAL;
     hipLaunchKernelGGL((resample_bwd_coef_staged_kernel<STAGED_TPW>), dim3((unsigned)(nb * N)), dim3(256), 0, s, gout, vol, bstride, coef,
                        partial, (int)nb, D, H, W, ntx, nty, ntz, p.st);
+    if (nblk_out != nullptr) *nblk_out = (int)nb;
     return bwd_coef_finish(partial, (int)nb, gcoef, N, s);
   }
   if (g_resample_variant >= 2 && p.vec && C == 16 && p.vpb >= 64 && p.nvox * 64 < 0xffffffffL) {
@@ -1012,6 +1005,7 @@
   } else {
     hipLaunchKernelGGL((resample_bwd_coef_kernel<1>), p.grid, dim3(256), 0, s, gout, vol, bstride, coef, partial, p.nblk, p.vpb, p.bt, N, D, H, W, C, p.lpv, p.st);
   }
+  if (nblk_out != nullptr) *nblk_out = p.nblk;
   return bwd_coef_finish(partial, p.nblk, gcoef, N, s);
 }
 
@@ -1020,6 +1014,14 @@
                                       int N, int D, int H, int W, int C, void* stream) {
   lf_clear_error();
   return bwd_coef_launch(gout, vol, vol_n, coef, gcoef, scratch, scratch_bytes, N, N, D, H, W, C, stream);
+}
+
+extern "C" int lf_resample3d_bwd_coef_partials(const float* gout, const float* vol, int vol_n, const float* coef,
+                                               void* scratch, size_t scratch_bytes,
+                                               int N, int D, int H, int W, int C, int* nblk, void* stream) {
+  lf_clear_error();
+  if (!gout || !vol || !coef || !scratch || !nblk) return LF_EINVAL;
+  return bwd_coef_launch(gout, vol, vol_n, coef, nullptr, scratch, scratch_bytes, N, N, D, H, W, C, stream, nblk);
 }
 
 extern "C" int lf_resample3d_bwd_coef_part(const float* gout, const float* vol, int vol_n, const float* coef,
@@ -1129,6 +1131,7 @@
   }
   if (key == 3) return lf_internal_fused_set_cfg(value);
   if (key == 5) return lf_internal_ring_bf16_set_wgs(value);
+  if (key == 7) return lf_internal_proj_stream_set_cfg(value);
   if (key == 2) {
     const int prev = g_bwd_coef_variant;
     if (value >= 1 && value <= 11) g_bwd_coef_variant = value;
diff --git a/latentfusion_amd/csrc/resample_partials.h b/latentfusion_amd/csrc/resample_partials.h
--- /dev/null
+++ b/latentfusion_amd/csrc/resample_partials.h
@@ -0,0 +1,18 @@
+#pragma once
+
+constexpr int LF_COEF_PARTIAL = 18;
+constexpr int LF_COEF_SUM_GROUPS = 14;
+
+__device__ __forceinline__ double lf_coef_partials_sum(const float* __restrict__ partial, int nblk, int n, double* red) {
+  const int comp = threadIdx.x % LF_COEF_PARTIAL;
+  const int grp = threadIdx.x / LF_COEF_PARTIAL;
+  double s = 0.0;
+  if (grp < LF_COEF_SUM_GROUPS)
+    for (int b = grp; b < nblk; b += LF_COEF_SUM_GROUPS) s += (double)partial[((long)n * nblk + b) * LF_COEF_PARTIAL + comp];
+  red[threadIdx.x] = (grp < LF_COEF_SUM_GROUPS) ? s : 0.0;
+  __syncthreads();
+  double tot = 0.0;
+  if (threadIdx.x < LF_COEF_PARTIAL)
+    for (int g = 0; g < LF_COEF_SUM_GROUPS; ++g) tot += red[g * LF_COEF_PARTIAL + threadIdx.x];
+  return tot;
+}
diff --git a/latentfusion_amd/engine.py b/latentfusion_amd/engine.py
--- a/latentfusion_amd/engine.py
+++ b/latentfusion_amd/engine.py
@@ -1,5 +1,6 @@
 import collections
 import contextlib
+import ctypes
 import math
 
 import torch
@@ -263,6 +264,9 @@
     EXPLICIT_DECODER = True
     EXPLICIT_OCCLUSION = True
     PROJ_GEMM = True
+    STREAM_PROJ_BWD = True
+    FUSED_FINISH = True
+    readback = None
 
     @staticmethod
     def supports(photographer, loss_weights):
@@ -386,11 +390,15 @@
         zt = z_target_latent if (z_target_latent is not None and self.w_latent != 0.0) else None
         if zt is not None and zt.shape[0] == 1 and n > 1:
             zt = zt.expand(n, *zt.shape[1:])
+        self.readback = None
         with _frozen(self._params):
             return self._run(params, intr, float(camera.z_span), need_grad, zt, masked_depth)
 
     def _run(self, params, intr, z_span, need_grad, zt, masked_depth):
-        return self._forward_backward_group(params, intr, z_span, need_grad, 1.0, zt, masked_depth)
+        rows = torch.empty(params.shape[0], 16, device=self.dev, dtype=torch.float32) if need_grad and self.FUSED_FINISH else None
+        out = self._forward_backward_group(params, intr, z_span, need_grad, 1.0, zt, masked_depth, rows=rows)
+        self.readback = rows
+        return out
 
     @staticmethod
     def _plan_occlusion(om):
@@ -506,7 +514,7 @@
                   'lf_occ_input_bwd')
         return gz
 
-    def _forward_backward_group(self, params, intr, z_span, need_grad, grad_scale, zt=None, masked_depth=False):
+    def _forward_backward_group(self, params, intr, z_span, need_grad, grad_scale, zt=None, masked_depth=False, rows=None):
         n = params.shape[0]
         flags = LF_EPI_LRELU | LF_EPI_PIXELNORM
         coefs, jac, cf20 = self._coefficients(params, intr, z_span, n)
@@ -550,7 +558,7 @@
         g, first, bounds = self._tail_bwd(tail, gp, g_leaf, acts, norms, flags, n)
         for i in range(first, -1, -1):
             g = self.plan.data_grad(i, g, acts, norms, flags, bounds)
-        return self._finish_backward(g, g_cf, cf20, jac, n, grad_scale, losses)
+        return self._finish_backward(g, g_cf, cf20, jac, n, grad_scale, losses, params, rows)
 
     def _coefficients(self, params, intr, z_span, n):
         L = _lib.lib()
@@ -635,10 +643,16 @@
         bounds = self.plan.grad_bounds()
         if self.plan.folds_prev:
             with ops._timed('factor_project_bwd'):
-                check(L.lf_conv1x1_bwd_data(gp.data_ptr(), ppack_t.data_ptr(), g.data_ptr(), n, S * S, cout, S * Cl,
-                                            S * S * S * Cl, Cl, Cl, S * S * Cl, phe, acts[nconv].data_ptr(),
-                                            norms[nconv - 1].data_ptr(), flags, ops.SLOPE,
-                                            bounds[nconv].data_ptr() if bounds is not None else None, _s()), 'lf_conv1x1_bwd_data')
+                if self.STREAM_PROJ_BWD and Cl == 16 and cout == 16 and bounds is None:
+                    check(L.lf_proj16_bwd_f32(gp.data_ptr(), ppack_t.data_ptr(), g.data_ptr(), acts[nconv].data_ptr(),
+                                              norms[nconv - 1].data_ptr(), n, S, S * S, phe, flags, ops.SLOPE, _s()),
+                          'lf_proj16_bwd_f32')
+                else:
+                    check(L.lf_conv1x1_bwd_data(gp.data_ptr(), ppack_t.data_ptr(), g.data_ptr(), n, S * S, cout, S * Cl,
+                                                S * S * S * Cl, Cl, Cl, S * S * Cl, phe, acts[nconv].data_ptr(),
+                                                norms[nconv - 1].data_ptr(), flags, ops.SLOPE,
+                                                bounds[nconv].data_ptr() if bounds is not None else None, _s()),
+                          'lf_conv1x1_bwd_data')
         else:
             ops._conv1x1_raw(gp, ppack_t, None, n, S * S, cout, 1, S * S * cout, 0, S * Cl, g, phe, 0,
                              yaddr=(S * S * S * Cl, Cl, Cl, S * S * Cl))
@@ -770,14 +784,31 @@
             check(L.lf_resample3d_bwd_coef(g.data_ptr(), self.z.data_ptr(), 1, cf20.data_ptr(), gcoef18.data_ptr(),
                                            scratch.data_ptr(), scratch.numel() * 4, n, S, S, S, self.C, _s()), 'lf_resample3d_bwd_coef')
 
-    def _finish_backward(self, g, g_cf, cf20, jac, n, grad_scale, losses):
+    def _finish_backward(self, g, g_cf, cf20, jac, n, grad_scale, losses, params=None, rows=None):
         L = _lib.lib()
         dev, s = self.dev, _s()
+        gparams = torch.empty(n, NPAR, device=dev, dtype=torch.float32)
+        gcoefs = g_cf.contiguous()
+        if self.FUSED_FINISH:
+            S = self.S
+            nbytes = L.lf_resample3d_bwd_coef_scratch_bytes(n, S, S, S)
+            scratch = torch.empty(nbytes // 4 + 1, device=dev, dtype=torch.float32)
+            nblk = ctypes.c_int(0)
+            with ops._timed('resample_bwd_coef'):
+                check(L.lf_resample3d_bwd_coef_partials(g.data_ptr(), self.z.data_ptr(), 1, cf20.data_ptr(), scratch.data_ptr(),
+                                                        scratch.numel() * 4, n, S, S, S, self.C, ctypes.addressof(nblk), s),
+                      'lf_resample3d_bwd_coef_partials')
+            if rows is not None:
+                losses, params = losses.contiguous(), params.contiguous()
+                assert losses.shape == (n, 8) and params.shape == (n, NPAR) and losses.dtype == params.dtype == torch.float32
+            check(L.lf_coef_grad_finish(scratch.data_ptr(), nblk.value, gcoefs.data_ptr(), jac.data_ptr(), gparams.data_ptr(),
+                                        float(grad_scale), losses.data_ptr() if rows is not None else None,
+                                        params.data_ptr() if rows is not None else None,
+                                        rows.data_ptr() if rows is not None else None, n, s), 'lf_coef_grad_finish')
+            return losses, gparams
         gcoef18 = torch.empty(n, 18, device=dev, dtype=torch.float32)
         self._bwd_coef(g, cf20, gcoef18, n)
-        gcoefs = g_cf.contiguous()
         gcoefs[:, :18] = gcoef18
-        gparams = torch.empty(n, NPAR, device=dev, dtype=torch.float32)
         check(L.lf_camera_coefs_bwd(gcoefs.data_ptr(), jac.data_ptr(), gparams.data_ptr(), n, s), 'lf_camera_coefs_bwd')
         if grad_scale != 1.0:
             gparams *= grad_scale
diff --git a/latentfusion_amd/engine_multi.py b/latentfusion_amd/engine_multi.py
--- a/latentfusion_amd/engine_multi.py
+++ b/latentfusion_amd/engine_multi.py
@@ -35,6 +35,7 @@
 class MultiTargetEngine(RenderLoopEngine):
 
     MAX_ROWS = 65535
+    FUSED_FINISH = False
 
     def __init__(self, photographer, z_obj, targets, loss_weights, conv_mode='auto', fuse_projection=None):
         targets = list(targets)
diff --git a/latentfusion_amd/pose/estimation.py b/latentfusion_amd/pose/estimation.py
--- a/latentfusion_amd/pose/estimation.py
+++ b/latentfusion_amd/pose/estimation.py
@@ -565,11 +565,14 @@
             z_target_latent = None
             if optim_weights.get('latent', 0.0) != 0.0 or self.loss_weights.get('latent', 0.0) != 0.0:
                 z_target_latent = self.model.compute_latent_code(st['target'], st['cam'])
+            dev = None
             if self.engine_graph and z_target_latent is None and not self.loss_schedules and hasattr(eng, 'forward_backward_graph'):
                 losses, gparams = eng.forward_backward_graph(st['cam'], P)
             else:
                 losses, gparams = eng.forward_backward(st['cam'], need_grad=True, z_target_latent=z_target_latent, params=P)
-            dev = torch.cat((losses[:, :6], P.detach()), dim=1)
+                dev = getattr(eng, 'readback', None)
+            if dev is None:
+                dev = torch.cat((losses[:, :6], P.detach()), dim=1)
             if st.get('shard') is not None:
                 from .. import parallel
                 dev = parallel.gather_rows(dev.contiguous(), st['shard'][2])
```

Measured after the change: 186.7. About the same (-0.4%).
